# CMU-SAFARI/PyGim

Measured on AMD Instinct MI355X. Metric: SpMM GFLOP/s, Reddit-shaped CSR h=256 fp32, higher is better.
Workload: dtype f32

## Files before the change

### pygim_amd/autotune.py

```python
from __future__ import annotations

import math
from dataclasses import dataclass

RATE_PANEL = 17.0e12
RATE_GATHER_FAR = 4.8e12
RATE_GATHER_MALL = 7.0e12
RATE_STREAM = 5.0e12
XGMI_IN = 7 * 45e9
PANEL_BYTES = 4 << 20
LAUNCH = 6e-6
CUS = 256
LDS_ROWS_MAX = 8 * 228
LDS_NS_PER_COLUMN = 3.43
LDS_NS_PER_ENTRY = 0.26
LDS_NS_PER_ENTRY_HALF = 0.5
LDS_NS_PER_COLUMN_FLOOR = 4.4
LDS_COL_SPLIT = True
LDS_ROW_TAIL = 3
TAIL_S = 30e-6
LDS_MIN_LANES = 5
LDS_MIN_REUSE_NARROW = 0.75
LDS_HALF_SPLIT = True
LDS_MIN_REUSE = 0.75


@dataclass
class Choice:
    row_parts: int
    feat_parts: int
    seconds: float
    product_s: float
    collective_s: float
    panel: bool


def lds_rows_per_tile(nrows, nslices, rmax=LDS_ROWS_MAX, cus=CUS):
    tiles = -(-nrows // rmax)
    wgs = tiles * nslices
    rounds = -(-wgs // cus)
    if rounds > 8:
        return rmax
    if wgs % cus == 0:
        return -(-nrows // tiles)
    tiles2 = rounds * cus // nslices
    if tiles2 <= tiles:
        return rmax
    return min(rmax, max(16, -(-nrows // tiles2)))


def lds_product_seconds(nrows, ncols, nnz, h, es):
    if es != 4 or h < LDS_MIN_LANES or nrows == 0 or nnz == 0:
        return None
    nsl = -(-h // 64)
    pack_s = ncols * h * es * 2 / RATE_STREAM
    cols_x = ncols
    ns_entry = LDS_NS_PER_ENTRY
    if LDS_HALF_SPLIT and h * es <= 128 and ncols >= 4 * 128:
        cols_x = -(-ncols // 2)
        ns_entry = LDS_NS_PER_ENTRY_HALF
    min_reuse = LDS_MIN_REUSE if h * es > 128 else max(LDS_MIN_REUSE, LDS_MIN_REUSE_NARROW * (1.6 if cols_x != ncols else 1.0))
    tall = -(-int(nrows) // LDS_ROWS_MAX)
    split = min(8, CUS // (tall * nsl)) if tall * nsl * 2 <= CUS else 1
    tail_rows = 0
    if LDS_COL_SPLIT and nnz >= (1 << 20):
        for s2 in range(8, split, -1):
            tall_s = CUS // (nsl * s2)
            if not tall_s:
                continue
            covered = tall_s * LDS_ROWS_MAX
            if covered >= nrows:
                break
            if (nrows - covered) * 100 <= nrows * LDS_ROW_TAIL and tall_s * nsl * s2 * 10 >= CUS * 9:
                split, tall, tail_rows = s2, tall_s, nrows - covered
                break
    if LDS_COL_SPLIT and nnz >= (1 << 20) and split > 1:
        if nnz / (tall * cols_x) < min_reuse:
            return None
        tall2 = CUS // (nsl * split)
        if not tail_rows and tall < tall2 <= 2 * tall:
            tall = tall2
        per_wg = max(cols_x / split * LDS_NS_PER_COLUMN + nnz / tall / split * ns_entry, cols_x / split * LDS_NS_PER_COLUMN_FLOOR) * 1e-9
        reduce_s = (split + 1) * nrows * h * es / RATE_STREAM
        return per_wg + reduce_s + pack_s + 2 * LAUNCH + (TAIL_S if tail_rows else 0.0)
    rpt = lds_rows_per_tile(int(nrows), nsl)
    tiles = -(-int(nrows) // rpt)
    if nnz / (tiles * cols_x) < min_reuse:
        return None
    per_wg = max(cols_x * LDS_NS_PER_COLUMN + nnz / tiles * ns_entry, cols_x * LDS_NS_PER_COLUMN_FLOOR) * 1e-9
    rounds = -(-tiles * nsl // CUS)
    return rounds * per_wg + pack_s + LAUNCH


def product_seconds(nrows, ncols, nnz, h, es):
    if nrows == 0 or nnz == 0 or h == 0:
        return 0.0, False
    t_lds = lds_product_seconds(nrows, ncols, nnz, h, es)
    if t_lds is not None:
        return t_lds, True
    row_bytes = h * es
    line_bytes = max(row_bytes, 128) if row_bytes < 128 else row_bytes
    gather = nnz * line_bytes
    npanels = max(1, math.ceil(ncols * 128 / PANEL_BYTES))
    panel = row_bytes >= 64 and (npanels == 1 or nnz / (nrows * npanels) >= 8)
    if panel:
        nsl = math.ceil(row_bytes / 128)
        t = gather / RATE_PANEL + npanels * (2 * nrows * row_bytes) / RATE_STREAM / 8 + nsl * 4 * nnz / RATE_STREAM / 8
        t += npanels * LAUNCH + ncols * row_bytes * 2 / RATE_STREAM
    else:
        x_bytes = ncols * row_bytes
        rate = RATE_GATHER_MALL if x_bytes <= 300e6 else RATE_GATHER_FAR
        t = gather / rate + LAUNCH
    return t, panel


def price(nrows, ncols, nnz, h, es, row_parts, feat_parts):
    hp = math.ceil(h / feat_parts)
    t, panel = product_seconds(math.ceil(nrows / row_parts), ncols, nnz / row_parts, hp, es)
    gpus = row_parts * feat_parts
    coll = 0.0 if gpus == 1 else (nrows * h * es) * (1 - 1 / gpus) / XGMI_IN
    return Choice(row_parts, feat_parts, t + coll, t, coll, panel)


def choose(nrows, ncols, nnz, h, elem_bytes, n_gpus):
    table = []
    for r in range(1, n_gpus + 1):
        if n_gpus % r:
            continue
        f = n_gpus // r
        if f > h:
            continue
        table.append(price(nrows, ncols, nnz, h, elem_bytes, r, f))
    best = min(table, key=lambda c: c.seconds)
    return best, table


def autotune(nrows, ncols, nnz, hidden_size, elem_bytes=4, n_gpus=8):
    best, _ = choose(nrows, ncols, nnz, hidden_size, elem_bytes, n_gpus)
    return [best.row_parts, best.feat_parts, "nnz", "nnz", None]


def autotune_dataset(datadir, dataset, hidden_size, split_set, blnc_set=(0, 2), elem_bytes=4):
    from . import datasets, synth

    assert len(split_set) > 0 and len(blnc_set) > 0
    got = datasets.load_adjacency(datadir, dataset)
    if got is not None:
        nrows, nnz = int(got[2]), int(len(got[1]))
    else:
        nrows, nnz, _ = synth.DATASETS[dataset]
    best = None
    for sp, ds in split_set:
        if sp < 1 or ds < 1 or ds > hidden_size:
            continue
        c = price(nrows, nrows, nnz, hidden_size, elem_bytes, sp, ds)
        if best is None or c.seconds < best.seconds:
            best = c
    if best is None:
        return [None, None, None, None, None]
    return [best.row_parts, best.feat_parts, "nnz", "nnz", None]
```

### pygim_amd/csrc/kernels.hpp

```cpp
#pragma once
#include <hip/hip_runtime.h>
#include <stdint.h>
#include <type_traits>

namespace pygim {

template <typename T> struct AccOf { using type = T; };
template <> struct AccOf<int8_t> { using type = uint32_t; };
template <> struct AccOf<int16_t> { using type = uint32_t; };
template <> struct AccOf<int32_t> { using type = uint32_t; };
template <> struct AccOf<int64_t> { using type = uint64_t; };

template <typename T> __device__ __forceinline__ typename AccOf<T>::type to_acc(T v) {
    using A = typename AccOf<T>::type;
    if constexpr (std::is_floating_point<T>::value) return v;
    else if constexpr (sizeof(T) == 8) return (A)v;
    else return (A)(int32_t)v;
}
template <typename T> __device__ __forceinline__ T from_acc(typename AccOf<T>::type a) {
    if constexpr (std::is_floating_point<T>::value) return a;
    else return (T)a;
}

__device__ __forceinline__ uint32_t rfl(uint32_t v) { return __builtin_amdgcn_readfirstlane(v); }
// ... 721 lines not shown
    const uint32_t f = (uint32_t)(i % w);
    using A = typename AccOf<T>::type;
    A acc = (A)part[r * ldp + f];
    for (uint32_t c = 1; c < splits; c++) acc = (A)(acc + (A)part[((uint64_t)c * nrows + r) * ldp + f]);
    float y = (float)(T)acc * (1.0f * quant_scale(*absmax_bits, log2_range));
    if (post_mul) {
        y = post_mul[f] * y + post_add[f];
        if (post_relu) y = fmaxf(y, 0.0f);
    }
    out[r * ldo + f] = y;
}

template <typename T, bool DEQ>
__global__ void k_lds_reduce_v4(const T *__restrict__ part, uint32_t splits, uint64_t nrows, uint32_t w, uint64_t ldp, void *__restrict__ C, int64_t ldc, int accumulate,
                                const uint32_t *__restrict__ absmax_bits, int log2_range, const float *__restrict__ post_mul, const float *__restrict__ post_add, int post_relu) {
    static_assert(sizeof(T) == 4, "4-byte element types");
    using A = typename AccOf<T>::type;
    const uint32_t w4 = w >> 2;
    const uint64_t i = (uint64_t)blockIdx.x * blockDim.x + threadIdx.x;
    if (i >= nrows * w4) return;
    const uint64_t r = i / w4;
    const uint32_t f = (uint32_t)(i % w4) * 4;
    T v[4];
    load_vec<T, 4>(part + r * ldp + f, v);
    A acc[4];
#pragma unroll
    for (int k = 0; k < 4; k++) acc[k] = to_acc<T>(v[k]);
    for (uint32_t c = 1; c < splits; c++) {
        load_vec<T, 4>(part + ((uint64_t)c * nrows + r) * ldp + f, v);
#pragma unroll
        for (int k = 0; k < 4; k++) acc[k] = (A)(acc[k] + to_acc<T>(v[k]));
    }
    if constexpr (DEQ) {
        const float scale = 1.0f * quant_scale(*absmax_bits, log2_range);
        float y[4];
#pragma unroll
        for (int k = 0; k < 4; k++) {
            y[k] = (float)from_acc<T>(acc[k]) * scale;
            if (post_mul) {
                y[k] = post_mul[f + k] * y[k] + post_add[f + k];
                if (post_relu) y[k] = fmaxf(y[k], 0.0f);
            }
        }
        store_vec<float, 4>((float *)C + r * ldc + f, y);
    } else {
        T *c = (T *)C + r * ldc + f;
        if (accumulate) {
            load_vec<T, 4>(c, v);
#pragma unroll
            for (int k = 0; k < 4; k++) acc[k] = (A)(to_acc<T>(v[k]) + acc[k]);
        }
#pragma unroll
        for (int k = 0; k < 4; k++) v[k] = from_acc<T>(acc[k]);
        store_vec<T, 4>(c, v);
    }
}

template <int MODE>
__global__ void k_lds_reduce16(const int16_t *__restrict__ part, uint32_t splits, uint64_t nrows, uint32_t w, uint64_t ldp, void *__restrict__ C, int64_t ldc, int accumulate,
                               const uint32_t *__restrict__ absmax_bits, int log2_range, const float *__restrict__ post_mul, const float *__restrict__ post_add, int post_relu) {
    const uint64_t i = (uint64_t)blockIdx.x * blockDim.x + threadIdx.x;
    if (i >= nrows * w) return;
    const uint64_t r = i / w;
    const uint32_t f = (uint32_t)(i % w);
    uint32_t acc = (uint32_t)(int32_t)part[r * ldp + f];
    for (uint32_t c = 1; c < splits; c++) acc += (uint32_t)(int32_t)part[((uint64_t)c * nrows + r) * ldp + f];
    if constexpr (MODE == 0) {
        int8_t *c8 = (int8_t *)C + (int64_t)r * ldc + f;
        if (accumulate) acc += (uint32_t)(int32_t)*c8;
        *c8 = (int8_t)acc;
    } else {
        float y = (float)(MODE == 1 ? (int32_t)(int8_t)acc : (int32_t)(int16_t)acc) * (1.0f * quant_scale(*absmax_bits, log2_range));
        if (post_mul) {
            y = post_mul[f] * y + post_add[f];
            if (post_relu) y = fmaxf(y, 0.0f);
        }
        ((float *)C)[(int64_t)r * ldc + f] = y;
    }
}

constexpr uint32_t LDS_TAIL_SEG = 256;
template <typename T>
__global__ __launch_bounds__(512) void k_lds_tail_seg(const uint32_t *__restrict__ segs, uint32_t nseg, const uint32_t *__restrict__ colind, const char *__restrict__ xs,
                                                      uint64_t slice_stride, typename AccOf<T>::type *__restrict__ parked) {
    static_assert(sizeof(T) == 4, "4-byte element types");
    using A = typename AccOf<T>::type;
    __shared__ A partial[8][64];
    const uint32_t seg = blockIdx.x, slice = blockIdx.y;
    const uint32_t wave = threadIdx.x >> 6, lane = threadIdx.x & 63;
    const uint32_t e0 = segs[nseg + seg], e1 = segs[2 * nseg + seg];
    const char *xsl = xs + (uint64_t)slice * slice_stride + lane * 4;
    static_assert(LDS_TAIL_SEG == 256, "32 entries per wave");
    uint32_t cols[32];
#pragma unroll
    for (int k = 0; k < 32; k++) {
        const uint32_t e = e0 + wave + 8u * k;
        cols[k] = e < e1 ? colind[e] : 0xFFFFFFFFu;
    }
    T x[32];
#pragma unroll
    for (int k = 0; k < 32; k++) x[k] = cols[k] != 0xFFFFFFFFu ? *(const T *)(xsl + (uint64_t)cols[k] * 256) : (T)0;
    A acc = 0;
#pragma unroll
    for (int k = 0; k < 32; k++) acc = (A)(acc + to_acc<T>(x[k]));
    partial[wave][lane] = acc;
    __syncthreads();
    if (wave != 0) return;
    A sum = partial[0][lane];
#pragma unroll
    for (int v = 1; v < 8; v++) sum = (A)(sum + partial[v][lane]);
    parked[((uint64_t)seg * gridDim.y + slice) * 64 + lane] = sum;
}
template <typename T, bool DEQ>
__global__ __launch_bounds__(64) void k_lds_tail_fin(const uint32_t *__restrict__ rowseg, uint32_t row0, const typename AccOf<T>::type *__restrict__ parked, uint32_t w_lanes,
                                                     void *__restrict__ C, int64_t ldc_bytes, int accumulate, const uint32_t *__restrict__ absmax_bits, int log2_range,
                                                     const float *__restrict__ post_mul, const float *__restrict__ post_add, int post_relu) {
    using A = typename AccOf<T>::type;
    const uint32_t t = blockIdx.x, slice = blockIdx.y, lane = threadIdx.x;
    const uint32_t f = slice * 64 + lane;
    if (f >= w_lanes) return;
    A sum = 0;
    for (uint32_t s = rowseg[t]; s < rowseg[t + 1]; s++) sum = (A)(sum + parked[((uint64_t)s * gridDim.y + slice) * 64 + lane]);
    const uint64_t row = (uint64_t)row0 + t;
    if constexpr (DEQ) {
        float y = (float)from_acc<T>(sum) * (1.0f * quant_scale(*absmax_bits, log2_range));
        if (post_mul) {
            y = post_mul[f] * y + post_add[f];
            if (post_relu) y = fmaxf(y, 0.0f);
        }
        *(float *)((char *)C + (int64_t)row * ldc_bytes + (size_t)f * 4) = y;
    } else {
        T *c = (T *)((char *)C + (int64_t)row * ldc_bytes + (size_t)f * 4);
        if (accumulate) sum = (A)(to_acc<T>(*c) + sum);
        *c = from_acc<T>(sum);
    }
}

__global__ void k_copy16(const u32x4_t *__restrict__ src, u32x4_t *__restrict__ dst, uint64_t n) {
    const uint64_t i = (uint64_t)blockIdx.x * blockDim.x + threadIdx.x;
    if (i < n) dst[i] = src[i];
}

template <typename T>
__global__ void k_narrow_vals(const T *__restrict__ vals, uint64_t n, typename NarrowOf<T>::type *__restrict__ narrow, int *flag) {
    using NT = typename NarrowOf<T>::type;
    const uint64_t i = (uint64_t)blockIdx.x * blockDim.x + threadIdx.x;
    if (i >= n) return;
    const T v = vals[i];
    const NT q = (NT)v;
    bool same;
    if constexpr (std::is_same<T, double>::value) same = __double_as_longlong((double)q) == __double_as_longlong(v);
    else same = (T)q == v;
    narrow[i] = q;
    if (!same) atomicOr(flag, 1);
}

template <typename T>
__global__ void k_widen_vals(const T *__restrict__ vals, uint64_t n, uint32_t *__restrict__ wide) {
    const uint64_t i = (uint64_t)blockIdx.x * blockDim.x + threadIdx.x;
    if (i < n) wide[i] = (uint32_t)(int32_t)vals[i];
}

template <typename T, int VEC, int LOG_LPR, int AMODE, int HAS_VALS, bool DEQ = false>
__global__ __launch_bounds__(256) void k_csr_panel(const uint32_t *__restrict__ item_row,
                                                   const uint32_t *__restrict__ item_begin,
                                                   const uint32_t *__restrict__ item_len, uint32_t nitems,
                                                   const uint32_t *__restrict__ coop_row,
                                                   const uint32_t *__restrict__ coop_begin,
                                                   const uint32_t *__restrict__ coop_len, uint32_t ncoop,
                                                   uint32_t coop_grid, const uint32_t *__restrict__ colind,
                                                   const T *__restrict__ vals, const T *__restrict__ X,
                                                   int64_t ldx, int64_t slice_stride, T *__restrict__ C,
                                                   int64_t ldc, uint32_t w, uint32_t nslices, int accumulate,
                                                   uint32_t col_base, float *__restrict__ Cf, int64_t ldcf,
                                                   const uint32_t *__restrict__ absmax_bits, int log2_range,
                                                   const float *__restrict__ post_mul, const float *__restrict__ post_add,
                                                   int post_relu) {
    static_assert(LOG_LPR == 3, "lane groups of 8 (one 128-byte line per gathered row slice)");
    if (blockIdx.x < coop_grid)
        panel_sweep<T, VEC, AMODE, HAS_VALS, true, DEQ>(blockIdx.x, coop_row, coop_begin, coop_len, ncoop, colind, vals, X,
                                                        ldx, slice_stride, C, ldc, w, nslices, accumulate, col_base, Cf, ldcf,
                                                        absmax_bits, log2_range, post_mul, post_add, post_relu);
    else
        panel_sweep<T, VEC, AMODE, HAS_VALS, false, DEQ>(blockIdx.x - coop_grid, item_row, item_begin, item_len, nitems,
// ... 675 lines not shown
```

### pygim_amd/csrc/lds_codegen.hpp

```cpp
#pragma once
#include <stdint.h>

#include <algorithm>
#include <stdexcept>
#include <vector>

#include "lds_plan.hpp"

#if defined(__HIPCC__)
#define PYGIM_HD __host__ __device__
#else
#define PYGIM_HD
#endif

namespace pygim {

struct CgParams {
    uint32_t NW = 8, KA = 228, KC = 128, NBUF = 5, RB = 256, RPB = 256, G = 10, NS = 2, XW = 1;
    uint32_t wide = 0, valued = 0;
    uint32_t mulw = 0;
    uint32_t int_inline = 0;
    uint32_t i64_full = 0;
    uint32_t opcode_add = 0x02000000u, addw = 1;
    uint32_t pieces = 4, chunk_bytes = 32768;
    uint32_t nrows = 0, ncols = 0, nchunks = 0, ntiles = 0, nstreams = 0;
    uint32_t S = 1, row_tiles = 0;
    uint32_t col_bits = 1;
    uint32_t half_H = 0;
    uint32_t x0 = 6, acc0 = 28, vbase0 = 1, vbase1 = 2, vbase2 = 3, vl16 = 4, vtouch = 4, vjunk = 5;
    uint32_t s_xs = 80, s_ldsw = 82, s_cb = 84, s_ret = 86, s_pa = 92;
    PYGIM_HD uint32_t vbase(uint32_t blk) const { return blk == 0 ? vbase0 : blk == 1 ? vbase1 : vbase2; }
};

constexpr uint32_t CG_TOUCH_EVERY_DW = 256;

inline CgParams cg_params(const LdsGeometry &geo, uint32_t opcode_add, bool valued, uint32_t nrows, uint32_t ncols, uint32_t gsize = 0, uint32_t nsets = 0,
                          bool int_inline = false, bool i64_full = false, uint32_t half_H = 0) {
    if (geo.NBUF >= 3 && !geo.boundary) throw std::runtime_error("lds codegen: the mid-slot hand-off takes the host encoder");
    CgParams P;
    const bool wide = geo.row_bytes == 512;
    if (geo.row_bytes != 256 && geo.row_bytes != 512) throw std::runtime_error("lds codegen: rows of 256 or 512 bytes");
    if (wide != (opcode_add == LDS_CODE_ADD_F64 || opcode_add == LDS_CODE_ADD_U64)) throw std::runtime_error("lds codegen: 512-byte rows are the 8-byte element types'");
    const LdsCodeRegs R = lds_code_regs(geo.NW, gsize, nsets, wide);
    P.NW = geo.NW; P.KA = geo.KA; P.KC = geo.KC; P.NBUF = geo.NBUF; P.RB = geo.row_bytes; P.RPB = 65536 / geo.row_bytes;
    P.G = R.gsize; P.NS = R.nsets; P.XW = wide ? 2 : 1; P.wide = wide; P.valued = valued;
    if (R.x0 + R.nx() > R.acc0 || R.acc0 + P.KA * P.XW > 256 || P.G > 12 || (P.NS - 1) * P.G > 15 || P.NS > 8)
        throw std::runtime_error("lds codegen: the geometry does not fit the register map");
    if (P.KA > 255) throw std::runtime_error("lds codegen: more than 255 accumulators per wave");
    P.opcode_add = opcode_add;
    P.i64_full = (valued && opcode_add == LDS_CODE_ADD_U64 && i64_full) ? 1 : 0;
    P.int_inline = (valued && (opcode_add == 0x68000000u || opcode_add == LDS_CODE_ADD_U64 || opcode_add == LDS_CODE_PK_ADD_U16) && int_inline && !P.i64_full) ? 1 : 0;
    P.mulw = !valued ? 0 : opcode_add == LDS_CODE_ADD_F64 ? 6 : opcode_add == LDS_CODE_ADD_U64 ? (P.i64_full ? 12 : P.int_inline ? 6 : 8) : ((opcode_add == 0x68000000u || opcode_add == LDS_CODE_PK_ADD_U16) && !int_inline) ? 4 : 2;
    P.addw = (opcode_add == LDS_CODE_PK_ADD_U16 || opcode_add == LDS_CODE_ADD_F64 || opcode_add == LDS_CODE_ADD_U64) ? 2 : 1;
    if (valued && opcode_add == LDS_CODE_ADD_U64) P.addw = 0;
    P.pieces = (geo.KC * geo.row_bytes / 1024) / geo.NW;
    if (P.pieces * geo.NW * 1024 != geo.KC * geo.row_bytes) throw std::runtime_error("lds codegen: a chunk is not a whole number of pieces per wave");
    P.chunk_bytes = geo.KC * geo.row_bytes;
    if ((geo.KC * geo.NBUF + P.RPB - 1) / P.RPB > 3) throw std::runtime_error("lds codegen: the ring is larger than three 64 KiB blocks");
    if (geo.NBUF > 12) throw std::runtime_error("lds codegen: more than 12 ring buffers");
    if ((geo.half_split != 0) != (half_H != 0)) throw std::runtime_error("lds codegen: a half-split plan names its H (and only such a plan does)");
    if (half_H && (valued || wide || half_H % geo.KC || ncols != half_H)) throw std::runtime_error("lds codegen: half-split plans are unit-weight plans of 4-byte types over H = whole chunks of virtual columns");
    P.half_H = half_H;
    P.nrows = nrows; P.ncols = ncols;
    P.nchunks = (ncols + geo.KC - 1) / geo.KC;
    const uint32_t R_rows = geo.rows_per_tile ? std::min(geo.rows_per_tile, geo.NW * geo.KA) : geo.NW * geo.KA;
    P.S = std::max(1u, geo.col_splits);
    P.row_tiles = (nrows + R_rows - 1) / R_rows;
    P.ntiles = P.row_tiles * P.S;
    P.nstreams = P.ntiles * geo.NW;
    if ((uint64_t)nrows * P.S >= (1ull << 32)) throw std::runtime_error("lds codegen: rows x column ranges beyond 32 bits");
    P.col_bits = 1;
    while (P.col_bits < 32 && (1ull << P.col_bits) < (uint64_t)ncols) P.col_bits++;
    uint32_t sb = 1;
    while ((1ull << sb) < (uint64_t)P.nstreams) sb++;
    if (sb + P.col_bits + 8 > 64) throw std::runtime_error("lds codegen: key wider than 64 bits");
    P.x0 = R.x0; P.acc0 = R.acc0; P.vbase0 = R.vbase[0]; P.vbase1 = R.vbase[1]; P.vbase2 = R.vbase[2];
    P.vl16 = R.vl16; P.vtouch = R.vtouch; P.vjunk = R.vjunk;
    P.s_xs = R.s_xs; P.s_ldsw = R.s_ldsw; P.s_cb = R.s_cb; P.s_ret = R.s_ret; P.s_pa = R.s_pa;
    return P;
}
inline uint32_t cg_key_bits(const CgParams &P) {
    uint32_t sb = 1;
    while ((1ull << sb) < (uint64_t)P.nstreams) sb++;
    return sb + P.col_bits + 8;
}

struct CgRows {
    std::vector<uint32_t> rowinfo;
    std::vector<uint32_t> rowmap_rt;
    std::vector<uint32_t> tnnz;
    std::vector<uint32_t> tile_pos;
    std::vector<uint32_t> rowmap;
    std::vector<uint32_t> tile_row0, tile_nnz;
};
inline void cg_deal_rows_a(const uint32_t *rowptr, const LdsGeometry &geo, const CgParams &P, CgRows &out, const uint32_t *rorder = nullptr) {
    auto rid = [&](uint32_t pos) { return rorder ? rorder[pos] : pos; };
    auto rlen = [&](uint32_t pos) { const uint32_t r = rid(pos); return rowptr[r + 1] - rowptr[r]; };
    const uint32_t NW = geo.NW, KA = geo.KA, KAS = geo.ka_stride(), RS = NW * KAS;
    const uint32_t R = geo.rows_per_tile ? std::min(geo.rows_per_tile, NW * KA) : NW * KA;
    const uint32_t nrows = P.nrows, nrt = P.row_tiles;
    out.rowinfo.assign(nrows, 0);
    out.rowmap_rt.assign((size_t)nrt * RS, 0xFFFFFFFFu);
    out.tnnz.assign((size_t)nrt * P.S, 0);
    lds_parallel_for(nrt, 0, [&](uint32_t rt) {
        std::vector<uint32_t> order;
        const uint32_t r0 = rt * R, r1 = std::min(nrows, r0 + R), nr = r1 - r0;
        if (P.S == 1) {
            if (!rorder) out.tnnz[rt] = rowptr[r1] - rowptr[r0];
            else
                for (uint32_t q = r0; q < r1; q++) out.tnnz[rt] += rlen(q);
        }
        order.resize(nr);
        for (uint32_t i = 0; i < nr; i++) order[i] = i;
        std::stable_sort(order.begin(), order.end(), [&](uint32_t a, uint32_t b) { return rlen(r0 + a) > rlen(r0 + b); });
        for (uint32_t i = 0; i < nr; i++) {
            const uint32_t round = i / NW, p = i % NW;
            const uint32_t w = (round & 1) ? NW - 1 - p : p;
            out.rowinfo[rid(r0 + order[i])] = ((rt * NW + w) << 8) | round;
            out.rowmap_rt[((size_t)rt * NW + w) * KAS + round] = rid(r0 + order[i]);
        }
    });
}
inline void cg_deal_rows_b(const LdsGeometry &geo, const CgParams &P, CgRows &out) {
    const uint32_t NW = geo.NW, KAS = geo.ka_stride(), RS = NW * KAS;
    const uint32_t R = geo.rows_per_tile ? std::min(geo.rows_per_tile, NW * geo.KA) : NW * geo.KA;
    const uint32_t ntiles = P.ntiles;
    std::vector<uint32_t> ord(ntiles);
    for (uint32_t t = 0; t < ntiles; t++) ord[t] = t;
    if (!geo.keep_tile_order) std::stable_sort(ord.begin(), ord.end(), [&](uint32_t a, uint32_t b) { return out.tnnz[a] > out.tnnz[b]; });
    out.tile_pos.assign(ntiles, 0);
    for (uint32_t i = 0; i < ntiles; i++) out.tile_pos[ord[i]] = i;
    out.rowmap.assign((size_t)ntiles * RS, 0xFFFFFFFFu);
    out.tile_row0.assign(ntiles, 0);
    out.tile_nnz.assign(ntiles, 0);
    for (uint32_t t = 0; t < ntiles; t++) {
        const uint32_t rt = t / P.S, cs = t % P.S, ti = out.tile_pos[t];
        out.tile_row0[ti] = rt * R;
        out.tile_nnz[ti] = out.tnnz[t];
        for (uint32_t q = 0; q < RS; q++) {
            const uint32_t r = out.rowmap_rt[(size_t)rt * RS + q];
            if (r != 0xFFFFFFFFu) out.rowmap[(size_t)ti * RS + q] = r + cs * P.nrows;
        }
    }
}

// ... 124 lines not shown
    }
    const uint32_t ch = T.chunks[T.choff[s / P.NW] + j];
    const uint64_t target = ((uint64_t)s << (P.col_bits + 8)) | ((uint64_t)ch * P.KC << 8);
    uint64_t lo = 0, hi = T.nnz;
    while (lo < hi) {
        const uint64_t mid = (lo + hi) >> 1;
        if (T.keys[mid] < target) lo = mid + 1;
        else hi = mid;
    }
    T.slot_firstcol[sj] = lo < T.nnz ? T.colx[lo] : T.ncols_total;
}
PYGIM_HD inline void cg_slot_ngroups(const CgParams &P, const CgTables &T, uint32_t sj) {
    const uint32_t m = T.slot_firstcol[sj + 1] - T.slot_firstcol[sj];
    T.slot_ng[sj] = (m + P.G - 1) / P.G;
}
PYGIM_HD inline unsigned long long cg_slot_groups(const CgParams &P, const CgTables &T, uint32_t sj) {
    const uint32_t c0 = T.slot_firstcol[sj], c1 = T.slot_firstcol[sj + 1];
    uint32_t g = T.slot_firstgroup[sj];
    unsigned long long pairs = 0;
    for (uint32_t c = c0; c < c1; c += P.G, g++) {
        const uint32_t ce = c + P.G < c1 ? c + P.G : c1;
        uint32_t nlds = 0;
        for (uint32_t u = 0; c + u < ce; u++) {
            T.col_g[c + u] = (g << 4) | u;
            if (P.wide) { nlds++; continue; }
            if ((u & 1) == 0) {
                const bool paired = c + u + 1 < c1 && (T.col_lrow[c + u + 1] / P.RPB) == (T.col_lrow[c + u] / P.RPB);
                if (paired) {
                    nlds++;
                    pairs += (unsigned long long)(T.col_first[c + u + 2] - T.col_first[c + u]);
                } else {
                    nlds += (c + u + 1 < ce) ? 2 : 1;
                }
            }
        }
        T.g_first[g] = T.col_first[c];
        T.g_nent[g] = T.col_first[ce] - T.col_first[c];
        if (P.half_H) {
            uint32_t n0 = 0;
            for (uint32_t i = T.col_first[c]; i < T.col_first[ce]; i++) n0 += T.vals[i] == 0u;
            T.g_n0[g] = n0;
        }
        T.g_firstcol[g] = c;
        T.g_nlds[g] = (uint8_t)nlds;
        T.g_ncols[g] = (uint8_t)(ce - c);
    }
    return pairs;
}

struct CgEmit {
    uint32_t *out;
    uint64_t n;
    uint32_t since_touch;
    uint64_t vm_touch;
    PYGIM_HD void put(uint32_t a) {
        if (out) out[n] = a;
        n++;
    }
    PYGIM_HD void op(uint32_t a) { put(a); since_touch++; }
    PYGIM_HD void op(uint32_t a, uint32_t b) { put(a); put(b); since_touch += 2; }
    PYGIM_HD void skip(uint32_t dw) { n += dw; since_touch += dw; }
};

PYGIM_HD inline void cg_stream_pass(const CgParams &P, const CgTables &T, uint32_t s, bool write) {
    const uint32_t ti = s / P.NW;
    const uint32_t nch = T.nch[ti];
    const uint32_t *chunk_ids = T.chunks + T.choff[ti];
    const uint32_t sj0 = cg_sbase(P, T, s);
    CgEmit e;
    const uint64_t base_dw = write ? T.start[s] / 4 : 0;
    e.out = write ? T.code + base_dw : nullptr;
    e.n = 0;
    e.since_touch = 0;
    e.vm_touch = 0;
    auto s_add_lit = [&](uint32_t sdst, uint32_t ssrc, uint32_t lit) { e.op(0x80000000u | (sdst << 16) | (0xFFu << 8) | ssrc, lit); };
    auto s_addc0 = [&](uint32_t sdst, uint32_t ssrc) { e.op(0x82000000u | (sdst << 16) | (0x80u << 8) | ssrc); };
    auto touch = [&]() {
        s_add_lit(P.s_cb, P.s_cb, (e.since_touch + 5) * 4);
        s_addc0(P.s_cb + 1, P.s_cb + 1);
        e.op(0xDC508000u, (P.vjunk << 24) | (P.s_cb << 16) | P.vtouch);
        e.since_touch = 0;
        e.vm_touch++;
    };
    auto dma = [&](uint32_t cid, uint32_t buf) {
        s_add_lit(P.s_pa, P.s_xs, cid * P.chunk_bytes);
        s_addc0(P.s_pa + 1, P.s_xs + 1);
        for (uint32_t i = 0; i < P.pieces; i++) {
            if (i % 4 == 0) {
                if (i) {
                    s_add_lit(P.s_pa, P.s_pa, 0x1000);
                    s_addc0(P.s_pa + 1, P.s_pa + 1);
                }
                s_add_lit(124 , P.s_ldsw, buf * P.chunk_bytes + (i / 4) * 0x1000);
                e.op(0xBF800000u);
            }
            e.op(0xDDF48000u | ((i % 4) * 1024), (P.s_pa << 16) | P.vl16);
        }
    };
    uint64_t dma_issued = 0;
    uint64_t landed_mark[16];
    for (int q = 0; q < 16; q++) landed_mark[q] = 0;
    auto vm_now = [&]() { return dma_issued + e.vm_touch; };
    auto dma_chunk = [&](uint32_t j) {
        dma(chunk_ids[j], j % P.NBUF);
        dma_issued += P.pieces;
        landed_mark[j & 15] = vm_now();
    };
    auto wait_landed = [&](uint32_t j) {
        const uint64_t younger = vm_now() - landed_mark[j & 15];
        const uint32_t nn = (uint32_t)(younger < 63 ? younger : 63);
        e.op(0xBF8C0F70u | (nn & 15) | (((nn >> 4) & 3) << 14));
    };
    auto wait_lgkm = [&](uint32_t n) { e.op(0xBF8CC07Fu | ((n < 15u ? n : 15u) << 8)); };
    uint32_t pend_g[10], pend_nlds[10], npend = 0;
    uint32_t gcount = 0;
    auto consume_oldest = [&]() {
        uint32_t younger = 0;
        for (uint32_t q = 1; q < npend; q++) younger += pend_nlds[q];
        wait_lgkm(younger);
        const uint32_t g = pend_g[0];
        if (write) T.g_apos[g] = (uint32_t)(base_dw + e.n);
        e.skip(T.g_nent[g] * (P.mulw + P.addw));
        if (P.half_H) e.skip((T.g_n0[g] > 0 ? 1u : 0u) + (T.g_n0[g] < T.g_nent[g] ? 1u : 0u) + 1u);
        for (uint32_t q = 1; q < npend; q++) {
            pend_g[q - 1] = pend_g[q];
            pend_nlds[q - 1] = pend_nlds[q];
        }
        npend--;
    };
    if (nch) {
        for (uint32_t j = 0; j + 1 < P.NBUF && j < nch; j++) dma_chunk(j);
        wait_landed(0);
        e.op(0xBF8A0000u);
    }
    for (uint32_t j = 0; j < nch; j++) {
        bool dma_due = j + P.NBUF - 1 < nch;
        const uint32_t g0 = T.slot_firstgroup[sj0 + j], g1 = T.slot_firstgroup[sj0 + j + 1];
        for (uint32_t g = g0; g < g1; g++) {
            const uint32_t nlds = T.g_nlds[g];
            if (write) {
                T.g_rpos[g] = (uint32_t)(base_dw + e.n);
                T.g_xset[g] = (uint8_t)(gcount % P.NS);
            }
            e.skip(2 * nlds);
            pend_g[npend] = g;
            pend_nlds[npend] = nlds;
            npend++;
            gcount++;
            if (dma_due) {
                dma_chunk(j + P.NBUF - 1);
                dma_due = false;
            }
            if (npend >= P.NS) consume_oldest();
            if (e.since_touch >= CG_TOUCH_EVERY_DW) touch();
        }
        if (dma_due) dma_chunk(j + P.NBUF - 1);
        while (npend > 1) consume_oldest();
        wait_lgkm(0);
        if (j + 1 < nch) wait_landed(j + 1);
        e.op(0xBF8A0000u);
    }
    while (npend) consume_oldest();
    e.op(0xBF8C0F70u);
    e.op(0xBE801D00u | P.s_ret);
    while (e.n % 64) e.put(0xBF800000u);
    if (!write) T.stream_dw[s] = (uint32_t)e.n;
}

PYGIM_HD inline void cg_emit_reads(const CgParams &P, const CgTables &T, uint32_t g) {
    if (P.half_H) {
        uint32_t *a = T.code + T.g_apos[g];
        const uint32_t n0 = T.g_n0[g], n1 = T.g_nent[g] - n0;
        uint32_t at = 0;
        if (n0) { a[at] = 0xBEFE0100u | 76u; at += 1 + n0 * P.addw; }
        if (n1) { a[at] = 0xBEFE0100u | 78u; at += 1 + n1 * P.addw; }
        a[at] = 0xBEFE01C1u;
    }
    const uint32_t c0 = T.g_firstcol[g], nc = T.g_ncols[g];
    const uint32_t xb = P.x0 + P.G * P.XW * T.g_xset[g];
    uint32_t *w = T.code + T.g_rpos[g];
    for (uint32_t u = 0; u < nc;) {
        const uint32_t r0 = T.col_lrow[c0 + u], blk = r0 / P.RPB;
        if (P.wide) {
            *w++ = 0xD8EC0000u | ((r0 % P.RPB) * P.RB);
            *w++ = ((xb + u * 2) << 24) | P.vbase(blk);
            u++;
        } else if ((u & 1) == 0 && u + 1 < nc && (T.col_lrow[c0 + u + 1] / P.RPB) == blk) {
            const uint32_t r1 = T.col_lrow[c0 + u + 1];
// ... 196 lines not shown
```

### pygim_amd/csrc/lds_plan.hpp

```cpp
#pragma once
#include <stdint.h>
#if defined(__HIPCC__)
#define PYGIM_LDS_HD_INLINE __host__ __device__ inline
#else
#define PYGIM_LDS_HD_INLINE inline
#endif

#include <algorithm>
#include <atomic>
#include <cstdio>
#include <cstdlib>
#include <memory>
#include <stdexcept>
#include <thread>
#include <vector>

namespace pygim {

struct LdsTile {
    uint32_t nch;
    uint32_t chunk_off;
    uint32_t nb_off;
    uint32_t row0;
    uint32_t nnz;
    uint32_t chunk0;
    uint32_t pad[2];
    uint32_t tokstart[16];
};

constexpr uint32_t LDS_TOK_SLACK = 4096 + 64;

constexpr uint32_t LDS_HDR_SHIFT = 18, LDS_HDR_MAX = 0x3FFFu;

struct LdsGeometry {
    uint32_t NW = 8;
    uint32_t KA = 208;
    uint32_t KC = 320;
    uint32_t BATCH = 16;
    uint32_t rows_per_tile = 0;
    uint32_t keep_tile_order = 0;
    uint32_t col_splits = 1;
    uint32_t ka_stride() const { return (KA + 7) & ~7u; }
    uint32_t row_bytes = 256;
    uint32_t boundary = 0;
    uint32_t half_split = 0;
    uint32_t NBUF = 2;
};

struct LdsPlanHost {
    LdsGeometry geo;
    uint32_t ntiles = 0, nchunks = 0;
    uint64_t ntokens = 0;
    uint64_t slots = 0;
    std::vector<uint32_t> tok;
    std::vector<uint32_t> wts;
    std::vector<uint32_t> nb, chunks, rowmap;
    std::vector<LdsTile> tiles;
    std::atomic<bool> header_overflow{false};
};

inline unsigned lds_default_threads() {
    static const unsigned cached = [] {
        unsigned hw = std::max(1u, std::thread::hardware_concurrency());
        long long quota = -1, period = 100000;
        if (FILE *f = fopen("/sys/fs/cgroup/cpu.max", "r")) {
            char q[32] = {0};
            if (fscanf(f, "%31s %lld", q, &period) == 2 && q[0] != 'm') quota = atoll(q);
            fclose(f);
        } else if (FILE *g = fopen("/sys/fs/cgroup/cpu/cpu.cfs_quota_us", "r")) {
            if (fscanf(g, "%lld", &quota) != 1) quota = -1;
            fclose(g);
            if (FILE *h = fopen("/sys/fs/cgroup/cpu/cpu.cfs_period_us", "r")) {
                if (fscanf(h, "%lld", &period) != 1) period = 100000;
                fclose(h);
            }
        }
        if (quota > 0 && period > 0) hw = (unsigned)std::min<long long>(hw, std::max<long long>(1, (quota + period - 1) / period));
        return hw;
    }();
    return cached;
}

template <typename F> inline void lds_parallel_for(uint32_t n, unsigned threads, F &&fn) {
    if (threads == 0) threads = lds_default_threads();
    threads = std::min<unsigned>(threads, std::max(1u, n));
    std::atomic<uint32_t> next(0);
    std::atomic<bool> failed(false);
    auto body = [&]() {
        try {
            for (;;) {
                const uint32_t i = next.fetch_add(1);
                if (i >= n || failed.load(std::memory_order_relaxed)) return;
                fn(i);
            }
        } catch (...) {
            failed.store(true);
        }
    };
    std::vector<std::thread> pool;
    try {
        for (unsigned i = 1; i < threads; i++) pool.emplace_back(body);
    } catch (...) {
    }
    body();
    for (auto &th : pool) th.join();
    if (failed.load()) throw std::runtime_error("lds plan: a worker failed (out of memory?)");
}

inline void lds_plan_build(const uint32_t *rowptr, const uint32_t *col, uint32_t nrows, uint32_t ncols, const LdsGeometry &geo,
                           LdsPlanHost &out, unsigned threads = 0, const uint32_t *vals = nullptr, const uint32_t *rorder = nullptr) {
    auto rid = [&](uint32_t pos) { return rorder ? rorder[pos] : pos; };
    auto rlen = [&](uint32_t pos) { const uint32_t r = rid(pos); return rowptr[r + 1] - rowptr[r]; };
    const uint32_t NW = geo.NW, KA = geo.KA, KC = geo.KC, B = geo.BATCH;
    const uint32_t KAS = geo.ka_stride();
    const uint32_t RS = NW * KAS;
    const uint32_t R = geo.rows_per_tile ? std::min(geo.rows_per_tile, NW * KA) : NW * KA;
    const uint32_t S = std::max(1u, geo.col_splits);
    const uint32_t ntiles = ((nrows + R - 1) / R) * S;
    const uint32_t nchunks = (ncols + KC - 1) / KC;
    out.geo = geo;
    out.ntiles = ntiles;
    out.nchunks = nchunks;
    out.tiles.assign(ntiles, LdsTile());
    out.rowmap.assign((size_t)ntiles * RS, 0xFFFFFFFFu);

    struct TileTmp {
        std::vector<uint32_t> chunk_ids;
        std::vector<uint32_t> cnt;
        std::vector<uint8_t> wave_of;
        std::vector<uint16_t> k_of;
        uint64_t batches[16] = {0, 0, 0, 0, 0, 0, 0, 0, 0, 0, 0, 0, 0, 0, 0, 0};
    };
    std::vector<TileTmp> tmp(ntiles);
    auto run = [&](auto &&fn) { lds_parallel_for(ntiles, threads, fn); };
    run([&](uint32_t t) {
        TileTmp &tt = tmp[t];
        const uint32_t rt = t / S, cs = t % S;
        const uint32_t ch_lo = (uint32_t)((uint64_t)nchunks * cs / S), ch_hi = (uint32_t)((uint64_t)nchunks * (cs + 1) / S);
        const uint32_t r0 = rt * R, r1 = std::min(nrows, r0 + R), nr = r1 - r0;
        std::vector<uint32_t> order(nr);
        for (uint32_t i = 0; i < nr; i++) order[i] = i;
        std::stable_sort(order.begin(), order.end(), [&](uint32_t a, uint32_t b) {
            return rlen(r0 + a) > rlen(r0 + b);
        });
        tt.wave_of.resize(nr);
        tt.k_of.resize(nr);
        for (uint32_t i = 0; i < nr; i++) {
            const uint32_t round = i / NW, pos = i % NW;
            const uint32_t w = (round & 1) ? NW - 1 - pos : pos;
            tt.wave_of[order[i]] = (uint8_t)w;
            tt.k_of[order[i]] = (uint16_t)round;
            out.rowmap[((size_t)t * NW + w) * KAS + round] = rid(r0 + order[i]) + cs * nrows;
        }
        std::vector<uint32_t> cnt((size_t)nchunks * NW, 0);
        for (uint32_t i = 0; i < nr; i++) {
            const uint32_t w = tt.wave_of[i];
            for (uint32_t e = rowptr[rid(r0 + i)]; e < rowptr[rid(r0 + i) + 1]; e++) {
                const uint32_t ch = col[e] / KC;
                if (ch >= ch_lo && ch < ch_hi) cnt[(size_t)ch * NW + w]++;
            }
        }
        uint32_t nnz_range = 0;
        for (uint32_t c = 0; c < nchunks; c++) {
            uint32_t any = 0;
            for (uint32_t w = 0; w < NW; w++) any |= cnt[(size_t)c * NW + w];
            if (!any) continue;
            tt.chunk_ids.push_back(c);
            for (uint32_t w = 0; w < NW; w++) {
                const uint32_t n = cnt[(size_t)c * NW + w];
                nnz_range += n;
                tt.cnt.push_back(n);
                tt.batches[w] += std::max<uint32_t>(1, (n + B - 1) / B);
            }
        }
        out.tiles[t].nch = (uint32_t)tt.chunk_ids.size();
        out.tiles[t].chunk0 = tt.chunk_ids.empty() ? 0 : tt.chunk_ids[0];
        out.tiles[t].row0 = r0;
        out.tiles[t].nnz = nnz_range;
    });
    uint64_t tokb = 0, nbo = 0, cho = 0, slots = 0;
    for (uint32_t t = 0; t < ntiles; t++) {
        LdsTile &d = out.tiles[t];
        d.chunk_off = (uint32_t)cho;
        d.nb_off = (uint32_t)nbo;
        cho += d.nch + 2;
        nbo += (uint64_t)(d.nch + 2) * NW;
        slots += d.nch;
        for (uint32_t w = 0; w < NW; w++) {
            d.tokstart[w] = (uint32_t)tokb;
            tokb += tmp[t].batches[w];
        }
    }
    out.slots = slots;
    out.ntokens = tokb * B;
    out.tok.assign((size_t)out.ntokens + LDS_TOK_SLACK, KA);
    if (vals) out.wts.assign(out.tok.size(), 0u);
    else out.wts.clear();
    out.nb.assign((size_t)nbo + 256, 0);
    out.chunks.assign((size_t)cho + 128, 0);
    run([&](uint32_t t) {
        TileTmp &tt = tmp[t];
        const LdsTile &d = out.tiles[t];
        const uint32_t rt = t / S, cs = t % S;
        const uint32_t r0 = rt * R, r1 = std::min(nrows, r0 + R), nr = r1 - r0, nch = d.nch;
        for (uint32_t j = 0; j < nch + 2; j++) out.chunks[(size_t)d.chunk_off + j] = nch ? tt.chunk_ids[std::min(j, nch - 1)] : 0;
// ... 25 lines not shown
                }
            }
        for (uint32_t w = 0; w < NW; w++) {
            uint64_t at = (uint64_t)d.tokstart[w] * B;
            for (uint32_t j = 0; j < nch; j++) {
                const uint32_t nbj = batches_of(j, w), nbn = batches_of(j + 1, w), cidn = j + 1 < nch ? tt.chunk_ids[j + 1] : 0;
                if (nbj > LDS_HDR_MAX || nbn > LDS_HDR_MAX || cidn > LDS_HDR_MAX) out.header_overflow = true;
                out.tok[at] |= nbj << LDS_HDR_SHIFT;
                out.tok[at + 1] |= nbn << LDS_HDR_SHIFT;
                out.tok[at + 2] |= cidn << LDS_HDR_SHIFT;
                at += (uint64_t)nbj * B;
            }
        }
        (void)nr;
    });
    std::vector<uint32_t> ord(ntiles);
    for (uint32_t t = 0; t < ntiles; t++) ord[t] = t;
    if (!geo.keep_tile_order) std::stable_sort(ord.begin(), ord.end(), [&](uint32_t a, uint32_t b) { return out.tiles[a].nnz > out.tiles[b].nnz; });
    std::vector<LdsTile> tiles2(ntiles);
    std::vector<uint32_t> rowmap2(out.rowmap.size());
    for (uint32_t i = 0; i < ntiles; i++) {
        tiles2[i] = out.tiles[ord[i]];
        std::copy(out.rowmap.begin() + (size_t)ord[i] * RS, out.rowmap.begin() + (size_t)(ord[i] + 1) * RS, rowmap2.begin() + (size_t)i * RS);
    }
    out.tiles.swap(tiles2);
    out.rowmap.swap(rowmap2);
}

inline uint32_t lds_rows_per_tile(uint32_t nrows, uint32_t rmax, uint32_t nslices, uint32_t cus) {
    if (!nrows || !nslices || !cus) return rmax;
    const uint64_t tiles = (nrows + rmax - 1) / rmax, wgs = tiles * nslices;
    const uint64_t rounds = (wgs + cus - 1) / cus;
    if (rounds > 8) return rmax;
    if (wgs % cus == 0) return (uint32_t)((nrows + tiles - 1) / tiles);
    const uint64_t tiles2 = rounds * cus / nslices;
    if (tiles2 <= tiles) return rmax;
    return (uint32_t)std::min<uint64_t>(rmax, std::max<uint64_t>(16, (nrows + tiles2 - 1) / tiles2));
}

inline double lds_plan_uniform_reuse(uint64_t nnz, uint32_t nrows, uint32_t ncols, const LdsGeometry &geo) {
    const uint64_t R = geo.rows_per_tile ? geo.rows_per_tile : (uint64_t)geo.NW * geo.KA;
    const uint64_t ntiles = (nrows + R - 1) / R;
    if (!ntiles || !ncols) return 0;
    return (double)nnz / ((double)ntiles * (double)ncols);
}


struct LdsCodeRegs {
    uint32_t vbase[3] = {0, 0, 0};
    uint32_t vl16 = 0;
    uint32_t vtouch = 0;
    uint32_t vjunk = 0;
    uint32_t x0 = 0;
    uint32_t gsize = 0, nsets = 0;
    uint32_t acc0 = 0;
    uint32_t s_xs = 80;
    uint32_t s_ldsw = 82;
    uint32_t s_cb = 84;
    uint32_t s_ret = 86;
    uint32_t s_pa = 92;
    uint32_t wide = 0;
    constexpr uint32_t nx() const { return gsize * nsets * (wide ? 2 : 1); }
};
constexpr LdsCodeRegs lds_code_regs(uint32_t NW, uint32_t gsize = 0, uint32_t nsets = 0, bool wide = false) {
    LdsCodeRegs r;
    r.wide = wide ? 1 : 0;
    if (NW == 16) {
        r.vbase[0] = 4; r.vbase[1] = 5; r.vbase[2] = 10;
        r.vl16 = 6; r.vtouch = 11; r.vjunk = 9; r.x0 = 12; r.acc0 = 28;
        r.gsize = gsize ? gsize : 8;
        r.nsets = nsets ? nsets : 2;
    } else {
        r.vbase[0] = 1; r.vbase[1] = 2; r.vbase[2] = 3;
        r.vl16 = 4; r.vtouch = 4; r.vjunk = 5; r.x0 = 6; r.acc0 = 28;
        r.gsize = gsize ? gsize : (wide ? 5 : 10);
        r.nsets = nsets ? nsets : 2;
    }
    if (!wide && (r.gsize & 1)) r.gsize--;
    if (r.gsize < 2) r.gsize = 2;
    if (r.nsets < 2) r.nsets = 2;
    while (r.x0 + r.nx() > r.acc0 && r.gsize > 2) r.gsize -= wide ? 1 : 2;
    return r;
}
constexpr uint32_t LDS_CODE_AUTO_WAVES = 8, LDS_CODE8_AUTO_NBUF = 5;
constexpr uint32_t LDS_CODE8_KA64 = 114;
constexpr uint32_t LDS_CODE8_KA = 228;

struct LdsWords {
    std::unique_ptr<uint32_t[]> p;
    size_t n = 0;
    void alloc(size_t words) { p.reset(new uint32_t[words]); n = words; }
    uint32_t *data() { return p.get(); }
    const uint32_t *data() const { return p.get(); }
    size_t size() const { return n; }
    uint32_t &operator[](size_t i) { return p[i]; }
    const uint32_t &operator[](size_t i) const { return p[i]; }
};

struct LdsCodeHost {
    LdsWords code;
    std::vector<uint64_t> start;
    uint64_t entries = 0;
    uint64_t pairs = 0;
    uint64_t shared = 0;
    LdsCodeRegs regs;
};

constexpr uint32_t LDS_CODE_PK_ADD_U16 = 0xFFFFFFFFu;
constexpr uint32_t LDS_CODE_ADD_F64 = 0xFFFFFFFEu, LDS_CODE_ADD_U64 = 0xFFFFFFFDu;
constexpr uint32_t LDS_CODE_S_VAL = 94;
inline bool lds_int_values_inline(const uint32_t *vals, uint64_t n) {
    for (uint64_t i = 0; i < n; i++) {
        const int32_t v = (int32_t)vals[i];
        if (v < -16 || v > 64) return false;
    }
    return true;
}
PYGIM_LDS_HD_INLINE uint32_t lds_inline_int(int32_t v) { return v >= 0 ? 128u + (uint32_t)v : 192u + (uint32_t)(-v); }
inline void lds_code_from_plan(const LdsPlanHost &plan, uint32_t opcode_add, LdsCodeHost &out, unsigned threads = 0, uint32_t gsize = 0,
                               uint32_t nsets = 0, uint32_t experiment = 0, const uint64_t *vals64 = nullptr) {
    const LdsGeometry &geo = plan.geo;
    const uint32_t NW = geo.NW, KA = geo.KA, B = geo.BATCH, KC = geo.KC;
    const uint32_t RB = geo.row_bytes;
    const bool wide = RB == 512;
    if (RB != 256 && RB != 512) throw std::runtime_error("lds code: rows of 256 or 512 bytes");
    if (wide != (opcode_add == LDS_CODE_ADD_F64 || opcode_add == LDS_CODE_ADD_U64)) throw std::runtime_error("lds code: 512-byte rows are the 8-byte element types'");
    if (!plan.wts.empty() && (opcode_add == LDS_CODE_ADD_F64 || opcode_add == LDS_CODE_ADD_U64) && !vals64)
        throw std::runtime_error("lds code: valued entries of this element type");
    const LdsCodeRegs R = lds_code_regs(NW, gsize, nsets, wide);
    out.regs = R;
    const uint32_t G = R.gsize, NS = R.nsets;
    if (R.x0 + R.nx() > R.acc0 || R.acc0 + KA * (wide ? 2 : 1) > 256 || G > 12 || (NS - 1) * G > 15)
        throw std::runtime_error("lds code: the geometry does not fit the register map");
    const uint32_t pieces = (KC * RB / 1024) / NW;
    if (pieces * NW * 1024 != KC * RB) throw std::runtime_error("lds code: a chunk is not a whole number of pieces per wave");
    const uint32_t chunk_bytes = KC * RB;
    const uint32_t RPB = 65536 / RB;
    if ((KC * geo.NBUF + RPB - 1) / RPB > 3) throw std::runtime_error("lds code: the ring is larger than three 64 KiB blocks");
    const uint32_t ntiles = plan.ntiles;
    constexpr uint32_t TOUCH_EVERY_DW = 256;

    struct Emit {
        uint32_t *out = nullptr;
        size_t n = 0;
        uint32_t since_touch = 0;
        uint64_t vm_touch = 0;
        void put(uint32_t a) {
            if (out) out[n] = a;
            n++;
        }
        void op(uint32_t a) { put(a); since_touch++; }
        void op(uint32_t a, uint32_t b) { put(a); put(b); since_touch += 2; }
    };
    struct Grp {
        uint32_t nx = 0, nlds = 0, xb = 0;
        std::vector<uint32_t> k, xr, v;
    };
    const LdsCodeRegs Rr = R;
    bool int_inline = (opcode_add == 0x68000000u || opcode_add == LDS_CODE_PK_ADD_U16) && !plan.wts.empty() && lds_int_values_inline(plan.wts.data(), plan.wts.size());
    bool i64_full = false;
    if (opcode_add == LDS_CODE_ADD_U64 && !plan.wts.empty()) {
        int_inline = true;
        for (uint64_t i = 0; i < plan.ntokens; i++) {
            if ((plan.tok[i] & 0xFF) >= KA) continue;
            const int64_t v = (int64_t)vals64[plan.wts[i]];
            if (v != (int64_t)(int32_t)v) i64_full = true;
            if (v < -16 || v > 64) int_inline = false;
        }
        if (i64_full) int_inline = false;
    }
    auto emit_stream = [&](uint32_t ti, uint32_t wv, Emit &e, uint64_t &n_entries, uint64_t &n_pairs, uint64_t &n_shared) {
        const LdsTile &t = plan.tiles[ti];
        auto s_add_lit = [&](uint32_t sdst, uint32_t ssrc, uint32_t lit) { e.op(0x80000000u | (sdst << 16) | (0xFFu << 8) | ssrc, lit); };
        auto s_addc0 = [&](uint32_t sdst, uint32_t ssrc) { e.op(0x82000000u | (sdst << 16) | (0x80u << 8) | ssrc); };
        auto touch = [&]() {
            s_add_lit(Rr.s_cb, Rr.s_cb, (e.since_touch + 5) * 4);
            s_addc0(Rr.s_cb + 1, Rr.s_cb + 1);
            e.op(0xDC508000u, (Rr.vjunk << 24) | (Rr.s_cb << 16) | Rr.vtouch);
            e.since_touch = 0;
            e.vm_touch++;
        };
        auto dma = [&](uint32_t cid, uint32_t buf) {
            s_add_lit(Rr.s_pa, Rr.s_xs, cid * chunk_bytes);
            s_addc0(Rr.s_pa + 1, Rr.s_xs + 1);
            for (uint32_t i = 0; i < pieces; i++) {
                if (i % 4 == 0) {
                    if (i) {
                        s_add_lit(Rr.s_pa, Rr.s_pa, 0x1000);
                        s_addc0(Rr.s_pa + 1, Rr.s_pa + 1);
                    }
                    s_add_lit(124 , Rr.s_ldsw, buf * chunk_bytes + (i / 4) * 0x1000);
                    e.op(0xBF800000u);
                }
                if (!(experiment & 2)) e.op(0xDDF48000u | ((i % 4) * 1024), (Rr.s_pa << 16) | Rr.vl16);
            }
        };
        uint64_t at = (uint64_t)t.tokstart[wv] * B;
        const uint32_t NBUF = geo.NBUF;
        const bool mid = NBUF >= 3 && !geo.boundary;
        uint64_t dma_issued = 0;
        auto vm_now = [&]() { return dma_issued + e.vm_touch; };
        std::vector<uint64_t> landed_mark(t.nch + NBUF + 1, 0);
        auto dma_chunk = [&](uint32_t j) {
            dma(plan.chunks[t.chunk_off + j], j % NBUF);
            dma_issued += (experiment & 2) ? 0 : pieces;
            landed_mark[j] = vm_now();
        };
        const bool spread = (experiment & 4) && pieces <= 4 && !mid;
        uint32_t dma_left = 0, dma_j = 0;
        auto dma_begin = [&](uint32_t j) {
            const uint32_t cid = plan.chunks[t.chunk_off + j], buf = j % NBUF;
            s_add_lit(Rr.s_pa, Rr.s_xs, cid * chunk_bytes);
            s_addc0(Rr.s_pa + 1, Rr.s_xs + 1);
            s_add_lit(124 , Rr.s_ldsw, buf * chunk_bytes);
            e.op(0xBF800000u);
            dma_left = pieces;
            dma_j = j;
        };
        auto dma_piece = [&]() {
            const uint32_t i = pieces - dma_left;
            e.op(0xDDF48000u | (i * 1024), (Rr.s_pa << 16) | Rr.vl16);
            dma_issued++;
            if (!--dma_left) landed_mark[dma_j] = vm_now();
        };
        auto wait_landed = [&](uint32_t j) {
            const uint64_t younger = vm_now() - landed_mark[j];
            const uint32_t nn = (uint32_t)std::min<uint64_t>(younger, 63);
            e.op(0xBF8C0F70u | (nn & 15) | (((nn >> 4) & 3) << 14));
        };
        auto wait_lgkm = [&](uint32_t n) { e.op(0xBF8CC07Fu | (std::min(n, 15u) << 8)); };
        const bool halves = geo.half_split != 0;
        const bool valued = !plan.wts.empty() && !halves;
        std::vector<Grp> ring(NS + 1);
        std::vector<uint32_t> pend;
        uint32_t gcount = 0;
        uint32_t lds_this_slot = 0;
        bool older_reads = false;
        auto consume_oldest = [&]() {
            uint32_t younger = 0;
            for (size_t q = 1; q < pend.size(); q++) younger += ring[pend[q]].nlds;
            wait_lgkm(younger);
            if (younger <= lds_this_slot) older_reads = false;
            const Grp &g = ring[pend.front()];
            if (valued && opcode_add == LDS_CODE_ADD_U64) {
                for (size_t q = 0; q < g.k.size(); q++) {
                    const uint64_t v64 = vals64[g.v[q]];
                    const int32_t v = (int32_t)(uint32_t)v64;
                    const uint32_t xl = g.xr[q], xh = g.xr[q] + 1, al = Rr.acc0 + g.k[q] * 2, ah = al + 1;
                    const uint32_t src = int_inline ? lds_inline_int(v) : LDS_CODE_S_VAL;
                    if (!int_inline) e.op(0xBE8000FFu | (LDS_CODE_S_VAL << 16), (uint32_t)v);
                    if (i64_full) e.op(0xBE8000FFu | ((LDS_CODE_S_VAL + 1) << 16), (uint32_t)(v64 >> 32));
                    e.op(0xD2850000u | xh, src | ((256 + xh) << 9));
                    if (!i64_full) e.op(v < 0 ? (0x6A000000u | (xh << 17) | (xl << 9) | (256 + xh)) : 0xBF800000u);
                    e.op(0x68000000u | (ah << 17) | (ah << 9) | (256 + xh));
                    if (i64_full) {
                        e.op(0xD2850000u | xh, (LDS_CODE_S_VAL + 1) | ((256 + xl) << 9));
                        e.op(0x68000000u | (ah << 17) | (ah << 9) | (256 + xh));
                    }
                    e.op(0xD1E86A00u | al, src | ((256 + xl) << 9) | ((256 + al) << 18));
                }
            } else if (valued && opcode_add == LDS_CODE_ADD_F64) {
                for (size_t q = 0; q < g.k.size(); q++) {
                    const uint64_t v = vals64[g.v[q]];
                    e.op(0xBE8000FFu | (LDS_CODE_S_VAL << 16), (uint32_t)v);
                    e.op(0xBE8000FFu | ((LDS_CODE_S_VAL + 1) << 16), (uint32_t)(v >> 32));
                    e.op(0xD2810000u | g.xr[q], LDS_CODE_S_VAL | ((256 + g.xr[q]) << 9));
                }
            } else if (valued && opcode_add == LDS_CODE_PK_ADD_U16) {
                for (size_t q = 0; q < g.k.size(); q++) {
                    if (!int_inline) e.op(0xBE8000FFu | (LDS_CODE_S_VAL << 16), g.v[q]);
                    e.op(0xD3814000u | g.xr[q], 0x10000000u | ((256 + g.xr[q]) << 9) | (int_inline ? lds_inline_int((int32_t)g.v[q]) : LDS_CODE_S_VAL));
                }
            } else if (valued && opcode_add == 0x68000000u) {
                for (size_t q = 0; q < g.k.size(); q++) {
                    if (int_inline) e.op(0xD2850000u | g.xr[q], lds_inline_int((int32_t)g.v[q]) | ((256 + g.xr[q]) << 9));
                    else {
                        e.op(0xBE8000FFu | (LDS_CODE_S_VAL << 16), g.v[q]);
                        e.op(0xD2850000u | g.xr[q], LDS_CODE_S_VAL | ((256 + g.xr[q]) << 9));
                    }
                }
            } else if (valued)
                for (size_t q = 0; q < g.k.size(); q++) e.op(0x0A0000FFu | (g.xr[q] << 17) | (g.xr[q] << 9), g.v[q]);
            for (uint32_t pass = 0; pass < (halves ? 2u : 1u); pass++) {
            if (halves) {
                bool any = false;
                for (size_t q = 0; q < g.k.size() && !any; q++) any = (g.v[q] & 1u) == pass;
                if (!any) continue;
                e.op(0xBEFE0100u | (pass ? 78u : 76u));
// ... 160 lines not shown
```

### pygim_amd/csrc/pygim_hip.hip

```cpp
#include "../../include/pygim_hip.h"
#include "kernels.hpp"
#ifdef PYGIM_LDS_ABLATE
#include "lds_kernel_gen_ablate.hpp"
#else
#include "lds_kernel_gen.hpp"
#include "lds_codegen_dev.hpp"
#include "lds_reorder_dev.hpp"
#include "lds_hybrid_dev.hpp"
#endif
#include "transpose_dev.hpp"
#include "sddmm_dev.hpp"
#include "spmm_values_dev.hpp"
#include "edge_softmax_dev.hpp"
#include <hsa/hsa.h>
#include <hsa/hsa_ext_amd.h>

static inline uint64_t lds_rows_pad(uint64_t ncols, uint32_t kc) {
    const uint64_t k = kc ? kc : 320;
    return ((ncols + k - 1) / k * k + 63) / 64 * 64;
}

#include <algorithm>
#include <atomic>
#include <chrono>
// ... 67 lines not shown
    }
    g_ctx.inited = false;
    g_ctx.generation++;
    return 0;
}

int64_t pygim_generation(void) { return g_ctx.generation; }

int pygim_device_info(char *name, int name_len, int *cu_count, int64_t *hbm_bytes) {
    int dev = 0;
    hipError_t e = hipGetDevice(&dev);
    if (e != hipSuccess) {
        (void)hipGetLastError();
        return fail(PYGIM_ERR_NO_DEVICE, "no HIP device visible");
    }
    hipDeviceProp_t prop;
    HIP_TRY(hipGetDeviceProperties(&prop, dev));
    if (name && name_len > 0) {
        std::snprintf(name, (size_t)name_len, "%s (%s)", prop.name, prop.gcnArchName);
    }
    if (cu_count) *cu_count = prop.multiProcessorCount;
    if (hbm_bytes) *hbm_bytes = (int64_t)prop.totalGlobalMem;
    return 0;
}

int64_t pygim_set_tunable(const char *name, int64_t value) {
    int64_t *slot = nullptr;
    std::string n = name ? name : "";
    if (n == "long_row_threshold") slot = &g_tune.long_row_threshold;
    else if (n == "long_segment") slot = &g_tune.long_segment;
    else if (n == "force_vec_bytes") slot = &g_tune.force_vec_bytes;
    else if (n == "csr_kernel") slot = &g_tune.csr_kernel;
    else if (n == "coo_chunk") slot = &g_tune.coo_chunk;
    else if (n == "coo_via_rowptr") slot = &g_tune.coo_via_rowptr;
    else if (n == "kernel_events") slot = &g_tune.kernel_events;
    else if (n == "host_windows") slot = &g_tune.host_windows;
    else if (n == "host_direct") slot = &g_tune.host_direct;
    else if (n == "panel_mode") slot = &g_tune.panel_mode;
    else if (n == "panel_bytes") slot = &g_tune.panel_bytes;
    else if (n == "panel_min_seg") slot = &g_tune.panel_min_seg;
    else if (n == "panel_pack") slot = &g_tune.panel_pack;
    else if (n == "panel_coop") slot = &g_tune.panel_coop;
    else if (n == "panel_block") slot = &g_tune.panel_block;
    else if (n == "slice_group_bytes") slot = &g_tune.slice_group_bytes;
    else if (n == "fuse_windows") slot = &g_tune.fuse_windows;
    else if (n == "panel_col16") slot = &g_tune.panel_col16;
    else if (n == "panel_locality") slot = &g_tune.panel_locality;
    else if (n == "split_unit_pattern") slot = &g_tune.split_unit_pattern;
    else if (n == "narrow_vals") slot = &g_tune.narrow_vals;
    else if (n == "merge_parts") slot = &g_tune.merge_parts;
    else if (n == "vec_kernel") slot = &g_tune.vec_kernel;
    else if (n == "vec_lds") slot = &g_tune.vec_lds;
    else if (n == "panel_lds_pad") slot = &g_tune.panel_lds_pad;
    else if (n == "vec_lds_min_seg") slot = &g_tune.vec_lds_min_seg;
    else if (n == "lds_mode") slot = &g_tune.lds_mode;
    else if (n == "lds_min_reuse_x100") slot = &g_tune.lds_min_reuse_x100;
    else if (n == "lds_min_width") slot = &g_tune.lds_min_width;
    else if (n == "lds_min_width8") slot = &g_tune.lds_min_width8;
    else if (n == "lds_min_reuse_narrow_x100") slot = &g_tune.lds_min_reuse_narrow_x100;
    else if (n == "lds_threads") slot = &g_tune.lds_threads;
    else if (n == "lds_waves") slot = &g_tune.lds_waves;
    else if (n == "lds_ablate") slot = &g_tune.lds_ablate;
    else if (n == "lds_round_tiles") slot = &g_tune.lds_round_tiles;
    else if (n == "lds_code") slot = &g_tune.lds_code;
    else if (n == "lds_code_nbuf") slot = &g_tune.lds_code_nbuf;
    else if (n == "lds_code_waves") slot = &g_tune.lds_code_waves;
    else if (n == "lds_fail") slot = &g_tune.lds_fail;
    else if (n == "lds_stamp") slot = &g_tune.lds_stamp;
    else if (n == "lds_code_exp") slot = &g_tune.lds_code_exp;
    else if (n == "lds_hybrid") slot = &g_tune.lds_hybrid;
    else if (n == "lds_hybrid_min") slot = &g_tune.lds_hybrid_min;
    else if (n == "lds_hybrid_contig") slot = &g_tune.lds_hybrid_contig;
    else if (n == "lds_code_boundary") slot = &g_tune.lds_code_boundary;
    else if (n == "lds_xcd_slices") slot = &g_tune.lds_xcd_slices;
    else if (n == "lds_codegen") slot = &g_tune.lds_codegen;
    else if (n == "lds_tile_order") slot = &g_tune.lds_tile_order;
    else if (n == "lds_lp_rounds") slot = &g_tune.lds_lp_rounds;
    else if (n == "lds_code_kc") slot = &g_tune.lds_code_kc;
    else if (n == "lds_code_gsize") slot = &g_tune.lds_code_gsize;
    else if (n == "lds_code_nsets") slot = &g_tune.lds_code_nsets;
    else if (n == "lds_col_split") slot = &g_tune.lds_col_split;
    else if (n == "lds_col_split_f32") slot = &g_tune.lds_col_split_f32;
    else if (n == "lds_fill_tiles") slot = &g_tune.lds_fill_tiles;
    else if (n == "lds_row_tail") slot = &g_tune.lds_row_tail;
    else if (n == "lds_split_order") slot = &g_tune.lds_split_order;
    else if (n == "lds_half_split") slot = &g_tune.lds_half_split;
    else if (n == "lds_direct_x") slot = &g_tune.lds_direct_x;
    else if (n == "lds_long_slots") slot = &g_tune.lds_long_slots;
    if (!slot) {
        fail(PYGIM_ERR_INVALID, "unknown tunable: " + n);
        return -1;
    }
    const int64_t old = *slot;
    if (slot == &g_tune.panel_lds_pad) value = std::min<int64_t>(std::max<int64_t>(value, 0), 64 << 10);
    *slot = value;
    return old;
}

}

static int group_create(int format, int dtype, int n_parts, const int32_t *const *idx0, const int32_t *const *colind,
                        const void *const *values, const int64_t *nrows, const int64_t *ncols, const int64_t *nnz,
                        const int64_t *n_dense, const int64_t *dense_cols, int64_t h_size, int64_t *out_handle, bool adopt) {
    bool adopted = false;
    auto drop_adopted = [&]() {
        if (!adopt || adopted) return;
        adopted = true;
        (void)hipFree(const_cast<int32_t *>(idx0[0]));
        (void)hipFree(const_cast<int32_t *>(colind[0]));
        if (values && values[0]) (void)hipFree(const_cast<void *>(values[0]));
    };
    if (int rc = need_init()) return drop_adopted(), rc;
    if (format != PYGIM_CSR && format != PYGIM_COO) return fail(PYGIM_ERR_INVALID, "format must be CSR(0) or COO(1)");
    const size_t es = dtype_size(dtype);
    if (es == 0) return fail(PYGIM_ERR_INVALID, "unknown dtype");
    if (n_parts <= 0 || !idx0 || !colind || !nrows || !ncols || !nnz || !n_dense || !dense_cols || !out_handle)
        return fail(PYGIM_ERR_INVALID, "null argument or n_parts <= 0");
    if (h_size <= 0) return fail(PYGIM_ERR_INVALID, "h_size must be positive");
    const double t0 = now_ms();
    Group *g = new Group;
    g->format = format;
    g->dtype = dtype;
    t_plan_dtype = dtype;
    g->h = h_size;
    g->total_rows = nrows[0];
    g->parts.resize(n_parts);
    hipStream_t st = nullptr;
    int rc = 0;
    auto bail = [&](int code) {
        (void)hipDeviceSynchronize();
        drop_adopted();
        free_group(g);
        return code;
    };
    if (hipMalloc((void **)&g->d_flags, 8 * sizeof(int)) != hipSuccess) return bail(fail(PYGIM_ERR_HIP, "hipMalloc flags"));
    if (hipMemsetAsync(g->d_flags, 0, 8 * sizeof(int), st) != hipSuccess) return bail(fail(PYGIM_ERR_HIP, "memset flags"));
    if (hipStreamCreateWithFlags(&g->side, hipStreamNonBlocking) != hipSuccess ||
        hipEventCreateWithFlags(&g->ev_fork, hipEventDisableTiming) != hipSuccess ||
        hipEventCreateWithFlags(&g->ev_join, hipEventDisableTiming) != hipSuccess)
        return bail(fail(PYGIM_ERR_HIP, "side stream / events"));
    size_t dpos = 0;
    for (int i = 0; i < n_parts; i++) {
        Part &p = g->parts[i];
        p.nrows = nrows[i];
        p.ncols = ncols[i];
        p.nnz = nnz[i];
        if (p.nrows != g->total_rows) return bail(fail(PYGIM_ERR_INVALID, "all sparse parts must have the same number of rows"));
        if (p.nrows < 0 || p.ncols < 0 || p.nnz < 0 || p.nnz > 0xFFFFFFFFll || p.nrows >= 0xFFFFFFFFll ||
            p.ncols > 0xFFFFFFFFll)
            return bail(fail(PYGIM_ERR_INVALID, "part sizes must fit 32-bit indices (the reference's uint32 matrices)"));
        if (n_dense[i] <= 0) return bail(fail(PYGIM_ERR_INVALID, "n_dense must be positive"));
        int64_t sum = 0;
        for (int64_t j = 0; j < n_dense[i]; j++) {
            if (dense_cols[dpos + j] < 0) return bail(fail(PYGIM_ERR_INVALID, "negative dense width"));
            p.dense_cols.push_back(dense_cols[dpos + j]);
            sum += dense_cols[dpos + j];
        }
        dpos += (size_t)n_dense[i];
        if (sum != h_size) return bail(fail(PYGIM_ERR_INVALID, "dense widths of a part must add up to h_size"));
        g->total_cols += p.ncols;
        if (!idx0[i] && (format == PYGIM_CSR || p.nnz > 0)) return bail(fail(PYGIM_ERR_INVALID, "null index array"));
        if (!colind[i] && p.nnz > 0) return bail(fail(PYGIM_ERR_INVALID, "null colind"));

        if ((rc = to_device<uint32_t>(colind[i], (size_t)p.nnz * 4, &p.colind, &p.own_colind, st))) return bail(rc);
        const void *v = values ? values[i] : nullptr;
        if (v) {
// ... 460 lines not shown
    out[1] = (int64_t)p.lds_slots;
    out[2] = (int64_t)p.lds_tokens;
    out[3] = p.nnz;
    return 0;
}

int pygim_group_lds_code(int64_t handle, int64_t out[4]) {
    Group *g = lookup(handle);
    if (!g) return fail(PYGIM_ERR_INVALID, "unknown group handle");
    const Part &p = (g->merged && g_tune.merge_parts && g->parts.size() > 1) ? *g->merged : g->parts[0];
    out[0] = p.lds_code ? (int64_t)p.lds_code_bytes : 0;
    out[1] = p.lds_code ? (int64_t)p.lds_code_pairs : 0;
    bool all_code = p.lds_is_code && g_tune.lds_code;
    if (!(g->merged && g_tune.merge_parts && g->parts.size() > 1))
        for (const Part &q : g->parts) all_code = all_code && q.lds_is_code;
    out[2] = all_code ? 1 : 0;
    out[3] = (p.lds_code && p.lds_codegen_device) ? 1 : 0;
    return 0;
}

int pygim_group_lds_tiles(int64_t handle, int64_t out[4]) {
    Group *g = lookup(handle);
    if (!g) return fail(PYGIM_ERR_INVALID, "unknown group handle");
    const Part &p = (g->merged && g_tune.merge_parts && g->parts.size() > 1) ? *g->merged : g->parts[0];
    out[0] = p.lds_tile_labels ? 1 : 0;
    out[1] = p.lds_tile_labels;
    out[2] = p.lds_tile_largest;
    out[3] = p.panel_locality_used ? p.sim_kind : 0;
    return 0;
}

int pygim_group_serial(int64_t handle, int64_t *out) {
    Group *g = lookup(handle);
    if (!g || !out) return fail(PYGIM_ERR_INVALID, "unknown group handle");
    *out = g->serial;
    return 0;
}

int pygim_group_lds_runs(int64_t handle, int64_t *out) {
    Group *g = lookup(handle);
    if (!g || !out) return fail(PYGIM_ERR_INVALID, "unknown group handle");
    *out = g->lds_runs;
    return 0;
}

int pygim_group_host_windows(int64_t handle, int64_t *windows, int64_t *direct) {
    Group *g = lookup(handle);
    if (!g || !windows) return fail(PYGIM_ERR_INVALID, "unknown group handle");
    *windows = g->host_windows_used;
    if (direct) *direct = g->host_direct_used;
    return 0;
}

int pygim_group_lds_geometry(int64_t handle, int64_t out[8]) {
    Group *g = lookup(handle);
    if (!g) return fail(PYGIM_ERR_INVALID, "unknown group handle");
    const Part &p = (g->merged && g_tune.merge_parts && g->parts.size() > 1) ? *g->merged : g->parts[0];
    for (int i = 0; i < 8; i++) out[i] = 0;
    if (!p.lds_tiles) return 0;
    out[0] = p.lds_nw;
    out[1] = p.lds_ka;
    out[2] = p.lds_kc;
    out[3] = p.lds_nbuf;
    out[4] = p.lds_is_code ? p.lds_code_gsize : 0;
    out[5] = p.lds_is_code ? p.lds_code_nsets : 0;
    out[6] = p.lds_is_code ? (int64_t)p.lds_code_shared : 0;
    out[7] = p.lds_col_splits;
    return 0;
}

int pygim_group_lds_note(int64_t handle, char *out, int64_t cap) {
    Group *g = lookup(handle);
    if (!g) return fail(PYGIM_ERR_INVALID, "unknown group handle");
    if (!out || cap <= 0) return fail(PYGIM_ERR_INVALID, "no buffer");
    std::string text;
    if ((g->merged && g_tune.merge_parts && g->parts.size() > 1) || g->parts.size() == 1) {
        text = ((g->merged && g_tune.merge_parts && g->parts.size() > 1) ? *g->merged : g->parts[0]).lds_note;
    } else {
        text = g->parts[0].lds_note;
        for (size_t i = 1; i < g->parts.size(); i++)
            if (g->parts[i].lds_note != g->parts[0].lds_note) text += "; part " + std::to_string(i) + ": " + g->parts[i].lds_note;
    }
    for (size_t i = 0; i < g->parts.size(); i++)
        if (!g->parts[i].hy_note.empty()) text += "; part " + std::to_string(i) + ": " + g->parts[i].hy_note;
    const size_t n = std::min<size_t>(text.size(), (size_t)cap - 1);
    std::memcpy(out, text.data(), n);
    out[n] = 0;
    return 0;
}

int pygim_group_info(int64_t handle, int64_t out[8]) {
    Group *g = lookup(handle);
    if (!g) return fail(PYGIM_ERR_INVALID, "unknown group handle");
    out[0] = g->total_rows;
    out[1] = g->total_cols;
    out[2] = g->h;
    out[3] = (int64_t)g->parts.size();
    int64_t nl = 0;
    for (auto &p : g->parts) nl += p.lp_base.n_long;
    out[4] = nl;
    out[5] = g->all_ones ? 1 : 0;
    out[6] = g->parts[0].d_items ? (int64_t)g->parts[0].npanels : 0;
    out[7] = (int64_t)g->parts[0].n_items;
    return 0;
}

int pygim_block_run_x(int64_t handle, int part, const void *X, int64_t ldx, void *C, int64_t ldc, int64_t width,
                      int accumulate, int x_unchanged, void *stream) {
    if (int rc = need_init()) return rc;
    Group *g = lookup(handle);
    if (!g) return fail(PYGIM_ERR_INVALID, "unknown group handle");
    if (part < 0 || part >= (int)g->parts.size()) return fail(PYGIM_ERR_INVALID, "part index out of range");
    if (!X || !C || width <= 0 || ldx < width || ldc < width) return fail(PYGIM_ERR_INVALID, "bad X/C/width/stride");
    if (!is_device_ptr(X) || !is_device_ptr(C)) return fail(PYGIM_ERR_INVALID, "pygim_block_run needs device pointers");
    g->x_unchanged = x_unchanged != 0;
    const int rc = launch_block_any(g, g->parts[part], X, ldx, C, ldc, width, accumulate != 0, (hipStream_t)stream);
    g->x_unchanged = false;
    return rc;
}

int pygim_block_run(int64_t handle, int part, const void *X, int64_t ldx, void *C, int64_t ldc, int64_t width,
                    int accumulate, void *stream) {
    return pygim_block_run_x(handle, part, X, ldx, C, ldc, width, accumulate, 0, stream);
}

int pygim_spmm_run_group_x(int64_t handle, const void *const *B_parts, void *out, int x_unchanged, void *stream) {
    if (int rc = need_init()) return rc;
    Group *g = lookup(handle);
    if (!g) return fail(PYGIM_ERR_INVALID, "unknown group handle");
    for (auto &p : g->parts)
        if (p.dense_cols != g->parts[0].dense_cols)
            return fail(PYGIM_ERR_INVALID, "spmm_run_group needs the same dense split for every sparse part");
    g->x_unchanged = x_unchanged != 0;
    const int rc = run_group_common(g, B_parts, nullptr, false, out, (hipStream_t)stream);
    g->x_unchanged = false;
    return rc;
}

int pygim_spmm_run_group(int64_t handle, const void *const *B_parts, void *out, void *stream) {
    return pygim_spmm_run_group_x(handle, B_parts, out, 0, stream);
}

int pygim_grande_run_group(int64_t handle, const void *const *B_windows, const int64_t *window_ld, void *out,
                           void *stream) {
    if (int rc = need_init()) return rc;
    Group *g = lookup(handle);
    if (!g) return fail(PYGIM_ERR_INVALID, "unknown group handle");
    if (!window_ld) return fail(PYGIM_ERR_INVALID, "window_ld is required");
    return run_group_common(g, B_windows, window_ld, true, out, (hipStream_t)stream);
}

int pygim_spmv_run_group(int64_t handle, const void *const *B_vectors, void *out, void *stream) {
    if (int rc = need_init()) return rc;
    Group *g = lookup(handle);
    if (!g) return fail(PYGIM_ERR_INVALID, "unknown group handle");
    hipStream_t st = (hipStream_t)stream;
    const size_t es = dtype_size(g->dtype);
    const size_t nvec = g->parts[0].dense_cols.size();
    for (auto &p : g->parts) {
        if (p.dense_cols.size() != nvec) return fail(PYGIM_ERR_INVALID, "spmv group: dense split differs between parts");
        for (auto wdt : p.dense_cols)
            if (wdt != 1) return fail(PYGIM_ERR_INVALID, "spmv group: every dense part must be one column wide");
    }
    if (!B_vectors || !out) return fail(PYGIM_ERR_INVALID, "null vectors or output");
    for (size_t j = 0; j < nvec; j++)
        if (!B_vectors[j]) return fail(PYGIM_ERR_INVALID, "null vector");
// ... 82 lines not shown
```

### pygim_amd/csrc/rt_launch.inc

```
int pick_vec_bytes(size_t es, const void *X, int64_t ldx, const void *C, int64_t ldc) {
    auto ok = [&](size_t vb) {
        return ((uintptr_t)X % vb == 0) && ((uintptr_t)C % vb == 0) && ((size_t)ldx * es % vb == 0) &&
               ((size_t)ldc * es % vb == 0);
    };
    size_t cap = g_tune.force_vec_bytes > 0 ? (size_t)g_tune.force_vec_bytes : 16;
    for (size_t vb : {(size_t)16, (size_t)8})
        if (vb <= cap && vb > es && ok(vb)) return (int)vb;
    return (int)es;
}

struct KernelTimer {
    Group *g;
    hipStream_t st;
    hipEvent_t a = nullptr, b = nullptr;
    KernelTimer(Group *g_, hipStream_t st_, bool on = true) : g(g_), st(st_) {
        if (on && (g_tune.kernel_events || g->kernel_events) && hipEventCreate(&a) == hipSuccess && hipEventCreate(&b) == hipSuccess)
            (void)hipEventRecord(a, st);
        else
            a = b = nullptr;
    }
    void stop() {
        if (!a) return;
        (void)hipEventRecord(b, st);
        g->ev_pending.emplace_back(a, b);
// ... 165 lines not shown
                       (AM == 3 ? (const uint32_t *)p.col16 : p.colind), vals, Xs0, ldg,                                  \
                       slice_stride, Cs0, ldc, ws, ns, (accumulate ? 1 : 0) | (p.panel_locality_used ? 2 : 0), q * p.panel_cols,   \
                       g->deq_out ? g->deq_out + (size_t)s0 * F : nullptr, g->deq_ld, g->deq_amax, g->deq_log2,                  \
                       g->post_mul ? g->post_mul + (size_t)s0 * F : nullptr, g->post_add ? g->post_add + (size_t)s0 * F : nullptr, \
                       g->post_relu)
#define PYGIM_LAUNCH_PANEL(AM, HV) PYGIM_LAUNCH_PANEL_D(AM, HV, false)
                int amode = !off32 ? 0 : ((size_t)ldg * sizeof(T) == 128 ? 2 : 1);
                if (amode == 2 && p.col16 && g_tune.panel_col16) amode = 3;
                if constexpr (DeqType<T>::ok) {
                    if (g->deq_out && amode >= 2 && !vals) {
                        if (amode == 3) PYGIM_LAUNCH_PANEL_D(3, 0, true);
                        else PYGIM_LAUNCH_PANEL_D(2, 0, true);
                        continue;
                    }
                }
                if (g->deq_out) return fail(PYGIM_ERR_INVALID, "internal: fused dequantisation on an unsupported sweep");
                if constexpr (sizeof(T) == 8) {
                    if (vals && p.vals_narrow && g_tune.narrow_vals) {
                        const T *vals = (const T *)p.vals_narrow;
                        if (amode == 3) PYGIM_LAUNCH_PANEL(3, 2);
                        else if (amode == 2) PYGIM_LAUNCH_PANEL(2, 2);
                        else if (amode == 1) PYGIM_LAUNCH_PANEL(1, 2);
                        else PYGIM_LAUNCH_PANEL(0, 2);
                        continue;
                    }
                }
                if (amode == 3 && vals) PYGIM_LAUNCH_PANEL(3, 1);
                else if (amode == 3) PYGIM_LAUNCH_PANEL(3, 0);
                else if (amode == 2 && vals) PYGIM_LAUNCH_PANEL(2, 1);
                else if (amode == 2) PYGIM_LAUNCH_PANEL(2, 0);
                else if (amode == 1 && vals) PYGIM_LAUNCH_PANEL(1, 1);
                else if (amode == 1) PYGIM_LAUNCH_PANEL(1, 0);
                else if (vals) PYGIM_LAUNCH_PANEL(0, 1);
                else PYGIM_LAUNCH_PANEL(0, 0);
#undef PYGIM_LAUNCH_PANEL
#undef PYGIM_LAUNCH_PANEL_D
            }
            }
            kt.stop();
            return join();
        }
    }
    bool wide = lanes_needed > 32;
    if (g_tune.csr_kernel == 1) wide = true;
    if (g_tune.csr_kernel == 2 && lanes_needed <= 32) wide = false;
    if (nrows > 0) {
        KernelTimer kt(g, st, !p.is_extra || p.timed);
        if (wide) {
            dim3 grid((nrows + 3) / 4, (lanes_needed + 63) / 64);
            hipLaunchKernelGGL((k_csr_wide<T, VEC>), grid, dim3(256), 0, st, p.rowptr, p.colind, vals, X, ldx, C,
                               ldc, nrows, w, lp.thresh, accumulate ? 1 : 0);
        } else {
            int log_lpr = 0;
            while ((1u << log_lpr) < lanes_needed) log_lpr++;
            const uint32_t rows_per_wave = 64u >> log_lpr;
            const uint32_t waves = (nrows + rows_per_wave - 1) / rows_per_wave;
            hipLaunchKernelGGL((k_csr_sub<T, VEC>), dim3((waves + 3) / 4), dim3(256), 0, st, p.rowptr, p.colind,
                               vals, X, ldx, C, ldc, nrows, w, lp.thresh, accumulate ? 1 : 0, log_lpr);
        }
        kt.stop();
    }
    return join();
}

template <typename T>
int launch_lds(Group *g, Part &p, const T *X, int64_t ldx, T *C, int64_t ldc, uint32_t w, bool accumulate, hipStream_t st,
               const void *lds_xs = nullptr, const uint32_t *deq_amax = nullptr, int deq_log2 = 0) {
    constexpr bool WIDE8 = sizeof(T) == 1;
    constexpr bool EL8 = sizeof(T) == 8;
    constexpr uint32_t ROWB = EL8 ? 512 : 256;
    constexpr uint32_t EPS = WIDE8 ? 128 : ROWB / sizeof(T);
    constexpr int PVEC = WIDE8 ? 8 : 16 / (int)sizeof(T);
    const bool split16 = p.lds_col_splits > 1 && (WIDE8 || (sizeof(T) == 2 && deq_amax != nullptr));
    const uint32_t w_lanes = split16 ? (uint32_t)(((size_t)w * 2 + 3) / 4)
                                     : (WIDE8 || EL8 || (sizeof(T) == 2 && deq_amax)) ? w : (uint32_t)(((size_t)w * sizeof(T) + 3) / 4);
    const bool HS = p.lds_half != 0;
    if (HS && (sizeof(T) != 4 || w > 32 || lds_xs || deq_amax)) return fail(PYGIM_ERR_INVALID, "internal: a half-split LDS plan serves plain 4-byte products of at most 32 lanes");
    const uint32_t nslices = HS ? 1u : (w + EPS - 1) / EPS;
    const uint64_t rows_pad = HS ? (uint64_t)p.lds_half : lds_rows_pad((uint64_t)p.ncols, p.lds_kc);
    const size_t need = (size_t)rows_pad * nslices * ROWB;
    KernelTimer kt(g, st, !p.is_extra || p.timed);
    XsPin pin;
    void *xs_use = const_cast<void *>(lds_xs);
    if (!xs_use && g_tune.lds_direct_x && nslices == 1 && !HS && !WIDE8 && !p.lds_col_order && (size_t)ldx * sizeof(T) == ROWB && (size_t)w * sizeof(T) == ROWB &&
        ((uintptr_t)X & 255) == 0) {
        void *base = nullptr;
        size_t size = 0;
        if (hipMemGetAddressRange((hipDeviceptr_t *)&base, &size, (hipDeviceptr_t)X) == hipSuccess && base && (const char *)X + (size_t)rows_pad * ROWB <= (const char *)base + size)
            xs_use = const_cast<void *>((const void *)X);
        else
            (void)hipGetLastError();
    }
    if (!xs_use) {
        std::lock_guard<std::mutex> lk(g_ctx.mu);
        if (g->x_unchanged) {
            int dev = 0;
            (void)hipGetDevice(&dev);
            Context::XsBuf *hit = nullptr;
            for (auto &kv : g_ctx.xs_bufs) {
                Context::XsBuf &b = kv.second;
                if (kv.first.first == dev && b.ptr && b.src == (const void *)X && b.ld == ldx && b.rows == p.ncols && b.w == (int64_t)w &&
                    b.es == sizeof(T) && b.kind == (HS ? 5 : WIDE8 ? 3 : 1) && b.rows_pad == rows_pad && b.order == (const void *)p.lds_col_order && b.bytes >= need &&
                    (!hit || b.stamp > hit->stamp))
                    hit = &b;
            }
            if (hit) {
                hit->stamp = ++g_ctx.xs_clock;
                hit->in_use++;
                xs_use = hit->ptr;
                pin.hold(xs_use);
            }
        }
        if (!xs_use) {
            Context::XsBuf *b = nullptr;
            if (int rc = xs_buffer_locked(st, std::max<size_t>(need, 256), &b)) return rc;
            xs_use = b->ptr;
            pin.hold(xs_use);
            b->src = X;
            b->ld = ldx;
            b->rows = p.ncols;
            b->w = (int64_t)w;
            b->es = sizeof(T);
            b->kind = HS ? 5 : WIDE8 ? 3 : 1;
            b->rows_pad = rows_pad;
            b->order = p.lds_col_order;
            const uint64_t threads = (uint64_t)p.ncols * nslices * 16;
            if (HS) {
                if constexpr (sizeof(T) == 4) {
                    const uint64_t th = rows_pad * 16;
                    hipLaunchKernelGGL((k_slice_pack_hs<T>), dim3((unsigned)((th + 255) / 256)), dim3(256), 0, st, X, ldx, (uint32_t)p.ncols, w, (uint32_t)rows_pad, (T *)xs_use);
                }
            } else if constexpr (WIDE8) {
                if (threads > 0)
                    hipLaunchKernelGGL(k_slice_pack_widen8, dim3((unsigned)((threads + 255) / 256)), dim3(256), 0, st, (const int8_t *)X, ldx,
                                       (uint32_t)p.ncols, w, nslices, (int16_t *)xs_use, (uint32_t)rows_pad, (const uint32_t *)p.lds_col_order);
            } else if constexpr (EL8) {
                const uint64_t th8 = (uint64_t)p.ncols * nslices * 32;
                if (th8 > 0)
                    hipLaunchKernelGGL((k_slice_pack<T, 2, 5>), dim3((unsigned)((th8 + 255) / 256)), dim3(256), 0, st, X, ldx,
                                       (uint32_t)p.ncols, w, nslices, (T *)xs_use, (uint32_t)rows_pad, (const uint32_t *)p.lds_col_order);
            } else if (threads > 0) {
                hipLaunchKernelGGL((k_slice_pack<T, PVEC, 4>), dim3((unsigned)((threads + 255) / 256)), dim3(256), 0, st, X, ldx,
                                   (uint32_t)p.ncols, w, nslices, (T *)xs_use, (uint32_t)rows_pad, (const uint32_t *)p.lds_col_order);
            }
        }
    }
    LdsArgs a{};
    a.tok = p.lds_tok;
    a.tiles = p.lds_tiles;
    a.rowmap = p.lds_rowmap;
    a.xs = (const char *)xs_use;
    a.c = (char *)C;
    a.slice_stride = rows_pad * ROWB;
    a.ldc_bytes = (uint32_t)((size_t)ldc * (((WIDE8 || sizeof(T) == 2) && deq_amax) ? 4 : sizeof(T)));
    a.w = w_lanes;
    a.nslices = nslices;
    a.ntiles = p.lds_ntiles;
    a.accumulate = accumulate ? 1 : 0;
    const uint32_t S = p.lds_col_splits;
    const uint64_t ldp = split16 ? (uint64_t)w_lanes * 2 : (uint64_t)w_lanes * 4 / sizeof(T);
    const size_t part_es = split16 ? 2 : sizeof(T);
    const uint64_t lds_rows = p.lds_rows ? p.lds_rows : (uint64_t)p.nrows;
    const bool deq_at_reduce = S > 1 && deq_amax != nullptr;
    if (S > 1) {
        const size_t need = (((size_t)S * (size_t)lds_rows * ldp * part_es + 255) & ~(size_t)255) + (size_t)p.lds_tail_nseg * nslices * 64 * 8;
        if (int rc = ensure(&g->scratch, &g->scratch_bytes, std::max<size_t>(need, 256))) return rc;
        a.c = (char *)g->scratch;
        a.ldc_bytes = (uint32_t)(ldp * part_es);
        a.accumulate = 0;
    }
    const uint32_t *kernel_amax = (deq_at_reduce || split16) ? nullptr : deq_amax;
    a.wdelta = p.lds_wdelta;
    a.deq_amax = kernel_amax;
    a.deq_log2 = deq_log2;
    a.post_mul = kernel_amax ? g->post_mul : nullptr;
    a.post_add = kernel_amax ? g->post_add : nullptr;
    a.post_relu = kernel_amax ? g->post_relu : 0;
    a.xcd_group = (nslices == 1 || nslices == 2 || nslices == 4 || nslices == 8) ? 8 / nslices : 0;
    a.xcd_sx = 1;
    if (a.xcd_group && p.lds_is_code && nslices > 1) {
        uint32_t sx = (uint32_t)std::max<int64_t>(0, g_tune.lds_xcd_slices);
        if (sx == 0) {
            const uint64_t nchunks = ((uint64_t)p.ncols + p.lds_kc - 1) / std::max(1u, p.lds_kc);
            const double fill = p.lds_ntiles && nchunks ? (double)p.lds_slots / ((double)p.lds_ntiles * (double)nchunks) : 1.0;
            sx = fill < 0.3 ? std::min(nslices, 4u) : (EL8 ? 1u : 2u);
        }
        if (sx > 1 && sx <= nslices && nslices % sx == 0) {
            a.xcd_sx = sx;
            a.xcd_group *= sx;
        }
    }
    a.half_split = HS ? 1u : 0u;
    a.xcd_contig = (a.xcd_group && p.lds_contig_tiles) ? (p.lds_ntiles + a.xcd_group - 1) / a.xcd_group : 0;
    const uint32_t grid = a.xcd_group ? 8 * ((p.lds_ntiles + a.xcd_group - 1) / a.xcd_group) * a.xcd_sx : p.lds_ntiles * nslices;
    using KernelFn = void (*)(LdsArgs);
    KernelFn fn = nullptr;
    const bool long16 = p.lds_nw == 16 && p.lds_batch == LDS_L16_BATCH;
    if (p.lds_is_code) {
        if (!g_tune.lds_code || g_tune.lds_ablate) return fail(PYGIM_ERR_INVALID, "this group's LDS plan is a code stream: lds_code was switched off (or lds_ablate on) after it was created");
        const bool w8 = p.lds_nw == 8;
        if constexpr (EL8) {
            if (!w8 || kernel_amax || S > 1 || p.lds_row_bytes != 512) return fail(PYGIM_ERR_INVALID, "internal: 8-byte LDS-staged product on an unsupported plan");
            if constexpr (std::is_same<T, double>::value) fn = k_lds_code8_f64;
            else fn = k_lds_code8_i64;
        } else if constexpr (sizeof(T) == 1) {
            if (!w8 || (accumulate && S <= 1)) return fail(PYGIM_ERR_INVALID, "internal: INT8 LDS-staged product on an unsupported plan");
            fn = split16 ? k_lds_code8_i16 : kernel_amax ? k_lds_code8_i8_deq : k_lds_code8_i8;
        } else if constexpr (sizeof(T) == 2) {
            if ((kernel_amax || split16) && !w8) return fail(PYGIM_ERR_INVALID, "internal: dequantising LDS-staged product on an unsupported plan");
            fn = kernel_amax ? k_lds_code8_i16_deq : (w8 ? k_lds_code8_i16 : k_lds_code_i16);
        } else if constexpr (std::is_same<T, float>::value) {
            fn = kernel_amax ? (w8 ? k_lds_code8_f32_deq : k_lds_code_f32_deq) : (w8 ? k_lds_code8_f32 : k_lds_code_f32);
        } else {
            fn = kernel_amax ? (w8 ? k_lds_code8_i32_deq : k_lds_code_i32_deq) : (w8 ? k_lds_code8_i32 : k_lds_code_i32);
        }
        if (g_tune.lds_stamp && fn == k_lds_code8_f32) {
            fn = k_lds_code8_f32_ts;
            a.stamps = (uint64_t *)(uintptr_t)g_tune.lds_stamp;
        }
        a.code = p.lds_code;
        a.code_start = p.lds_code_start;
        a.piece_bytes = p.lds_code_piece;
    } else if constexpr (sizeof(T) == 1 || sizeof(T) == 8) {
        return fail(PYGIM_ERR_INVALID, "internal: the INT8 / INT64 / DBL64 LDS-staged product exists in the code-stream form only");
    } else if (kernel_amax) {
        if (p.lds_nw != 16 || p.lds_wdelta || sizeof(T) != 4) return fail(PYGIM_ERR_INVALID, "internal: dequantising LDS-staged product on an unsupported plan");
        if constexpr (std::is_same<T, float>::value) fn = long16 ? k_lds_spmm_f32_w16b_deq : k_lds_spmm_f32_w16_deq;
        else if constexpr (std::is_same<T, int32_t>::value) fn = long16 ? k_lds_spmm_i32_w16b_deq : k_lds_spmm_i32_w16_deq;
    } else if constexpr (sizeof(T) == 2) {
        if (p.lds_nw != 16) return fail(PYGIM_ERR_INVALID, "internal: INT16 LDS-staged product needs the 16-wave plan");
        fn = long16 ? k_lds_spmm_i16_w16b : (p.lds_wdelta ? k_lds_spmm_i16_w16_val : k_lds_spmm_i16_w16);
    } else if (long16) {
        if constexpr (std::is_same<T, float>::value) fn = k_lds_spmm_f32_w16b;
        else fn = k_lds_spmm_i32_w16b;
    } else if constexpr (std::is_same<T, float>::value) {
        fn = p.lds_nw == 16 ? (p.lds_wdelta ? k_lds_spmm_f32_w16_val : k_lds_spmm_f32_w16) : k_lds_spmm_f32_w8;
#ifdef PYGIM_LDS_ABLATE
        if (p.lds_nw == 16 && !p.lds_wdelta && !long16) {
            switch (g_tune.lds_ablate) {
                case 6: fn = k_lds_spmm_f32_w16_ab6; break;
                case 7: fn = k_lds_spmm_f32_w16_ab7; break;
                case 10: fn = k_lds_spmm_f32_w16_ab10; break;
                case 11: fn = k_lds_spmm_f32_w16_ab11; break;
                case 12: fn = k_lds_spmm_f32_w16_ab12; break;
                case 15: fn = k_lds_spmm_f32_w16_ab15; break;
                case 16: fn = k_lds_spmm_f32_w16_ab16; break;
                case 17: fn = k_lds_spmm_f32_w16_ab17; break;
                case 18: fn = k_lds_spmm_f32_w16_ab18; break;
                case 19: fn = k_lds_spmm_f32_w16_ab19; break;
                default: break;
            }
        }
#else
        if (g_tune.lds_ablate) return fail(PYGIM_ERR_INVALID, "lds_ablate needs the ablation build (make -C pygim_amd/csrc ablate)");
#endif
    } else {
        fn = p.lds_nw == 16 ? (p.lds_wdelta ? k_lds_spmm_i32_w16_val : k_lds_spmm_i32_w16) : k_lds_spmm_i32_w8;
    }
    if (kernel_amax && g_tune.lds_ablate) return fail(PYGIM_ERR_INVALID, "lds_ablate is a timing experiment of the plain kernel");
    if (!fn) return fail(PYGIM_ERR_INVALID, "internal: no LDS-staged kernel for this plan");
    {
        static std::set<std::pair<int, KernelFn>> attr_done;
        int dev = 0;
        HIP_TRY(hipGetDevice(&dev));
        std::lock_guard<std::mutex> lk(g_ctx.mu);
        if (!attr_done.count({dev, fn})) {
            HIP_TRY(hipFuncSetAttribute((const void *)fn, hipFuncAttributeMaxDynamicSharedMemorySize, (int)LDS_BYTES));
            attr_done.insert({dev, fn});
        }
    }
    hipLaunchKernelGGL(fn, dim3(grid), dim3(p.lds_nw * 64), LDS_BYTES, st, a);
    g->lds_runs++;
    if (split16 && lds_rows > 0 && w > 0) {
        const uint64_t total = lds_rows * w;
        const dim3 rg((unsigned)((total + 255) / 256));
        if (!deq_amax)
            hipLaunchKernelGGL((k_lds_reduce16<0>), rg, dim3(256), 0, st, (const int16_t *)g->scratch, S, lds_rows, w, ldp, (void *)C, ldc, accumulate ? 1 : 0, nullptr, 0, nullptr, nullptr, 0);
        else if (WIDE8)
            hipLaunchKernelGGL((k_lds_reduce16<1>), rg, dim3(256), 0, st, (const int16_t *)g->scratch, S, lds_rows, w, ldp, (void *)C, ldc, 0, deq_amax, deq_log2, g->post_mul, g->post_add, g->post_relu);
        else
            hipLaunchKernelGGL((k_lds_reduce16<2>), rg, dim3(256), 0, st, (const int16_t *)g->scratch, S, lds_rows, w, ldp, (void *)C, ldc, 0, deq_amax, deq_log2, g->post_mul, g->post_add, g->post_relu);
    } else if (S > 1 && lds_rows > 0 && w > 0 && sizeof(T) == 4 && (w & 3) == 0 && (ldp & 3) == 0 && (ldc & 3) == 0 && ((uintptr_t)C & 15) == 0) {
        if constexpr (sizeof(T) == 4) {
            const uint64_t total4 = lds_rows * (w >> 2);
            const dim3 rg((unsigned)((total4 + 255) / 256));
            if (deq_at_reduce)
                hipLaunchKernelGGL((k_lds_reduce_v4<T, true>), rg, dim3(256), 0, st, (const T *)g->scratch, S, lds_rows, w, ldp, (void *)C, ldc, 0, deq_amax, deq_log2, g->post_mul,
                                   g->post_add, g->post_relu);
            else
                hipLaunchKernelGGL((k_lds_reduce_v4<T, false>), rg, dim3(256), 0, st, (const T *)g->scratch, S, lds_rows, w, ldp, (void *)C, ldc, accumulate ? 1 : 0, nullptr, 0, nullptr,
                                   nullptr, 0);
        }
    } else if (S > 1 && lds_rows > 0 && w > 0) {
        const uint64_t total = lds_rows * w;
        if constexpr (sizeof(T) == 4) {
            if (deq_at_reduce)
                hipLaunchKernelGGL((k_lds_reduce_deq<T>), dim3((unsigned)((total + 255) / 256)), dim3(256), 0, st, (const T *)g->scratch, S, lds_rows, w, ldp, (float *)C, ldc,
                                   deq_amax, deq_log2, g->post_mul, g->post_add, g->post_relu);
        }
        if (!deq_at_reduce)
            hipLaunchKernelGGL((k_lds_reduce<T>), dim3((unsigned)((total + 255) / 256)), dim3(256), 0, st, (const T *)g->scratch, S, lds_rows, w, ldp, C,
                               ldc, accumulate ? 1 : 0);
    }
    if (lds_rows < (uint64_t)p.nrows && w > 0) {
        if constexpr (sizeof(T) == 4) {
            using A = typename AccOf<T>::type;
            if (!p.lds_tail_segs || !p.lds_tail_rowseg) return fail(PYGIM_ERR_INVALID, "internal: an LDS plan that leaves rows out has no segment table for them");
            const uint32_t ntail = (uint32_t)((uint64_t)p.nrows - lds_rows);
            const size_t split_bytes = S > 1 ? (((size_t)S * (size_t)lds_rows * ldp * sizeof(T) + 255) & ~(size_t)255) : 0;
            const size_t park_bytes = (size_t)p.lds_tail_nseg * nslices * 64 * sizeof(A);
            if (int rc = ensure(&g->scratch, &g->scratch_bytes, std::max<size_t>(split_bytes + park_bytes, 256))) return rc;
            A *parked = (A *)((char *)g->scratch + split_bytes);
            if (p.lds_tail_nseg > 0)
                hipLaunchKernelGGL((k_lds_tail_seg<T>), dim3(p.lds_tail_nseg, nslices), dim3(512), 0, st, p.lds_tail_segs, p.lds_tail_nseg, p.colind, (const char *)xs_use,
                                   (uint64_t)(rows_pad * ROWB), parked);
            const int64_t ldc_b = (int64_t)ldc * 4;
            if (deq_amax)
                hipLaunchKernelGGL((k_lds_tail_fin<T, true>), dim3(ntail, nslices), dim3(64), 0, st, p.lds_tail_rowseg, (uint32_t)lds_rows, parked, w, (void *)C, ldc_b, 0, deq_amax,
                                   deq_log2, g->post_mul, g->post_add, g->post_relu);
            else
                hipLaunchKernelGGL((k_lds_tail_fin<T, false>), dim3(ntail, nslices), dim3(64), 0, st, p.lds_tail_rowseg, (uint32_t)lds_rows, parked, w, (void *)C, ldc_b,
                                   accumulate ? 1 : 0, nullptr, 0, nullptr, nullptr, 0);
        } else {
            return fail(PYGIM_ERR_INVALID, "internal: an LDS plan that leaves rows to the tail kernels exists for 4-byte element types only");
        }
    }
    kt.stop();
    HIP_TRY(hipGetLastError());
    return 0;
}

template <typename T> bool want_lds(const Group *g, const Part &p, uint32_t w, int64_t ldc, const void *C, bool accumulate = false) {
    if constexpr (sizeof(T) == 8) {
        if (!p.lds_is_code || p.lds_nw != 8 || p.lds_row_bytes != 512 || p.lds_col_splits > 1 || false) return false;
    } else if (p.lds_row_bytes == 512) return false;
    if constexpr (sizeof(T) == 1) {
        if (!p.lds_is_code || p.lds_nw != 8 || (accumulate && p.lds_col_splits <= 1)) return false;
        if ((int64_t)(w / 2) < g_tune.lds_min_width) return false;
    }
    if constexpr (sizeof(T) == 2) {
        if ((w & 1) || (ldc & 1) || ((uintptr_t)C & 3) || (p.lds_nw != 16 && !p.lds_is_code)) return false;
    }
    if (!p.lds_tiles || g_tune.lds_mode == 2 || (!p.lds_is_code && (p.vals != nullptr) != (p.lds_wdelta != 0)) || g->deq_out || g->pre_xs) return false;
    if (p.lds_half && (sizeof(T) != 4 || w > 32)) return false;
    if (p.lds_is_code && (!g_tune.lds_code || g_tune.lds_ablate)) return false;
    if (g_tune.lds_mode == 0 && (g_tune.panel_mode == 1 || g_tune.csr_kernel != 0 || g_tune.force_vec_bytes != 0)) return false;
    if (sizeof(T) > 1 && (int64_t)(sizeof(T) == 8 ? (size_t)w : (size_t)w * sizeof(T) / 4) < (sizeof(T) == 8 ? g_tune.lds_min_width8 : g_tune.lds_min_width)) return false;
    if ((uint64_t)ldc * sizeof(T) >= (1ull << 32)) return false;
    return true;
}

template <typename T>
int launch_block(Group *g, Part &p, const void *X, int64_t ldx, void *C, int64_t ldc, int64_t w, bool accumulate,
                 hipStream_t st) {
    const T *x = (const T *)X;
    T *c = (T *)C;
    const uint32_t ww = (uint32_t)w;
    if (want_lds<T>(g, p, ww, ldc, C, accumulate)) return launch_lds<T>(g, p, x, ldx, c, ldc, ww, accumulate, st);
    if (ww <= 4 && g_tune.vec_kernel && g_tune.force_vec_bytes == 0 && g_tune.csr_kernel == 0 && p.rowptr && p.nrows > 0) {
        using A = typename AccOf<T>::type;
        constexpr size_t LDS_TOTAL = 160 * 1024 - 64;
        const size_t panel_lds = (((((size_t)p.panel_cols + 1) * ww * sizeof(T)) + 15) & ~(size_t)15) + 16;
        const size_t per_entry = 4 + (size_t)ww * sizeof(A);
        const bool lds_rule = g_tune.vec_lds && g_tune.panel_mode != 2 && p.d_items && p.col16 && p.lp_panel.n_tasks == 0 && !p.panel_locality_used &&
                              p.npanels >= 1 && p.panel_long128.size() == 4 * (size_t)p.npanels && (uint64_t)p.nnz < (1ull << 31) &&
                              (double)p.nnz >= (double)g_tune.vec_lds_min_seg * (double)p.nrows * (double)p.npanels;
        if (lds_rule && panel_lds + 64 * 12 * per_entry <= LDS_TOTAL) {
            const size_t stage_budget = std::min<size_t>(32 * 1024, LDS_TOTAL - panel_lds);
            uint32_t F16 = (uint32_t)(stage_budget / (64 * per_entry)) / 24 * 24;
            const int merge4 = F16 == 0 ? 1 : 0;
            if (merge4) F16 = (uint32_t)(stage_budget / (64 * per_entry)) / 12 * 12;
            const size_t shmem = panel_lds + 64 * (size_t)F16 * per_entry;
            const uint32_t cu = (uint32_t)std::max(g_ctx.cu_count, 1);
            if (!p.d_spmv_units) {
                std::vector<uint32_t> act;
                double wsum = 0;
                for (uint32_t q = 0; q < p.npanels; q++)
                    if (p.panel_off[q + 1] > p.panel_off[q]) {
                        act.push_back(q);
                        wsum += (double)std::max<uint64_t>(p.panel_nnz[q], p.panel_off[q + 1] - p.panel_off[q]);
                    }
                if (!act.empty()) {
                    std::vector<uint32_t> nb(act.size(), 1);
                    if (act.size() < cu) {
                        uint32_t left = cu - (uint32_t)act.size();
                        std::vector<std::pair<double, size_t>> rem;
                        uint32_t given = 0;
                        for (size_t k = 0; k < act.size(); k++) {
                            const uint32_t q = act[k];
                            const double share = (double)left * (double)std::max<uint64_t>(p.panel_nnz[q], p.panel_off[q + 1] - p.panel_off[q]) / wsum;
                            const uint32_t fl = (uint32_t)share;
                            nb[k] += fl;
                            given += fl;
                            rem.emplace_back(share - fl, k);
                        }
                        std::sort(rem.begin(), rem.end(), [](const std::pair<double, size_t> &x, const std::pair<double, size_t> &y) { return x.first > y.first; });
                        for (size_t k = 0; given < left && k < rem.size(); k++, given++) nb[rem[k].second]++;
                    }
// ... 154 lines not shown
```

### pygim_amd/csrc/rt_plans.inc

```
template <typename T> void launch_check_ones(const void *v, uint32_t n, int *flag, hipStream_t st) {
    hipLaunchKernelGGL((k_check_ones<T>), dim3((n + 255) / 256), dim3(256), 0, st, (const T *)v, n, flag);
}

void plan_long_rows(const uint32_t *rowptr, int64_t nrows, uint32_t thresh, uint32_t seg, const std::vector<char> *flags,
                    std::vector<uint32_t> &tasks, std::vector<uint32_t> &desc) {
    for (int64_t r = 0; r < nrows; r++) {
        const uint32_t s = rowptr[r], e = rowptr[r + 1];
        const bool is_long = flags ? (*flags)[(size_t)r] != 0 : (e - s > thresh);
        if (!is_long || e == s) continue;
        const uint32_t first = (uint32_t)(tasks.size() / 3);
        uint32_t n = 0;
        for (uint32_t a = s; a < e; a += seg, n++) {
            tasks.push_back((uint32_t)r);
            tasks.push_back(a);
            tasks.push_back(std::min(e, a + seg));
        }
        desc.push_back((uint32_t)r);
        desc.push_back(first);
        desc.push_back(n);
    }
}

int build_lds_plan(Part &p, size_t es, int *d_flag_sorted, hipStream_t st, const std::vector<uint32_t> &h_rowptr, int64_t h_hint);
double now_ms();
// ... 426 lines not shown
    };
    const size_t val_es = es;
    const bool int8_code = es == 1 && t_plan_dtype == PYGIM_INT8 && allow_code && g_tune.lds_code && g_tune.lds_waves == 16 && g_tune.lds_code_waves != 16;
    if (es == 1) {
        if (!int8_code) return 0;
        es = 2;
    }
    const bool el8_code = es == 8 && (t_plan_dtype == PYGIM_INT64 || t_plan_dtype == PYGIM_DBL64) && allow_code && g_tune.lds_code &&
                          g_tune.lds_waves == 16 && g_tune.lds_code_waves != 16;
    if (es == 8 && !el8_code) return 0;
    if (g_tune.lds_mode == 2 || (es != 4 && es != 2 && es != 8) || p.is_extra || p.nnz == 0 || p.nrows == 0 || p.ncols == 0) return 0;
    if ((p.vals || es == 2) && g_tune.lds_waves != 16) return 0;
    if (h_hint > 0 && (es == 8 ? h_hint : (h_hint * (int64_t)std::max<size_t>(es, 2)) / 4) < (es == 8 ? g_tune.lds_min_width8 : g_tune.lds_min_width)) return 0;
    if ((uint64_t)p.ncols * (es == 8 ? 512ull : 256ull) >= (1ull << 32) - (1ull << 20) || (uint64_t)p.nnz >= (1ull << 31)) return 0;
    LdsGeometry geo;
    geo.NW = g_tune.lds_waves == 16 ? 16 : 8;
    geo.KA = lds_ka(geo.NW);
    geo.KC = LDS_KC;
    geo.BATCH = lds_batch(geo.NW);
    geo.keep_tile_order = p.lds_contig_tiles ? 1u : 0u;
    const bool want_code = allow_code && g_tune.lds_code && geo.NW == 16 &&
                           ((es == 4 && t_plan_dtype == PYGIM_FLT32) || (es == 4 && t_plan_dtype == PYGIM_INT32) ||
                            (es == 2 && t_plan_dtype == PYGIM_INT16) || int8_code || el8_code);
    const int64_t slice_b = es == 8 ? 512 : 256;
    const int64_t nsl_hint = h_hint > 0 ? (h_hint * (int64_t)es + slice_b - 1) / slice_b : 4;
    if (want_code) {
        const int64_t cw = g_tune.lds_code_waves;
        const bool eight = cw == 8 || (cw != 16 && LDS_CODE_AUTO_WAVES == 8) || int8_code || el8_code;
        if (eight) {
            geo.NW = 8;
            geo.KA = el8_code ? LDS_CODE8_KA64 : LDS_CODE8_KA;
            geo.BATCH = 8;
        }
        if (el8_code) geo.row_bytes = 512;
    }
    if (g_tune.lds_round_tiles && h_hint > 0)
        geo.rows_per_tile = lds_rows_per_tile((uint32_t)p.nrows, geo.NW * geo.KA, (uint32_t)nsl_hint, (uint32_t)std::max(g_ctx.cu_count, 1));
    const bool f32_split_ok = g_tune.lds_col_split_f32 == 1 ? p.nnz >= (1 << 20) : g_tune.lds_col_split_f32 != 0;
    uint32_t rows_lds = (uint32_t)p.nrows;
    if (g_tune.lds_col_split != 1 && (geo.NW == 16 || want_code) && !el8_code && (t_plan_dtype != PYGIM_FLT32 || f32_split_ok) && !p.vals) {
        const uint32_t cus = (uint32_t)std::max(g_ctx.cu_count, 1);
        const uint64_t nsl = h_hint > 0 ? (uint64_t)nsl_hint : 1;
        const uint64_t tall = ((uint64_t)p.nrows + geo.NW * geo.KA - 1) / (geo.NW * geo.KA), wgs = tall * nsl;
        uint32_t S = 1;
        if (g_tune.lds_col_split > 1) S = (uint32_t)std::min<int64_t>(g_tune.lds_col_split, 16);
        else if (wgs * 2 <= cus) S = (uint32_t)std::min<uint64_t>(8, cus / wgs);
        if (g_tune.lds_col_split == 0 && g_tune.lds_row_tail > 0 && want_code && es == 4 && !p.lds_forced && (uint64_t)p.nrows * 8 < (1ull << 31)) {
            const uint64_t full = (uint64_t)geo.NW * geo.KA;
            for (uint32_t S2 = 8; S2 > S; S2--) {
                const uint64_t tall2 = cus / (nsl * S2);
                if (!tall2) continue;
                const uint64_t covered = tall2 * full;
                if (covered >= (uint64_t)p.nrows) break;
                if (((uint64_t)p.nrows - covered) * 100 <= (uint64_t)p.nrows * (uint64_t)g_tune.lds_row_tail && tall2 * nsl * S2 * 10 >= (uint64_t)cus * 9) {
                    S = S2;
                    rows_lds = (uint32_t)covered;
                    break;
                }
            }
        }
        if (S > 1 && (uint64_t)p.nrows * S < (1ull << 31)) {
            geo.col_splits = S;
            geo.rows_per_tile = 0;
            if (g_tune.lds_split_order && (((uint64_t)rows_lds + geo.NW * geo.KA - 1) / (geo.NW * geo.KA)) * nsl * S <= cus) geo.keep_tile_order = 1;
            if (g_tune.lds_col_split == 0 && g_tune.lds_fill_tiles && rows_lds == (uint32_t)p.nrows) {
                const uint64_t tall2 = cus / (nsl * S);
                if (tall2 > tall && tall2 <= 2 * tall) geo.rows_per_tile = (uint32_t)std::max<uint64_t>(16, ((uint64_t)p.nrows + tall2 - 1) / tall2);
            }
        }
    }
    if (want_code) {
        code_ring(geo.NW, geo.row_bytes, geo.NBUF, geo.KC);
        geo.boundary = g_tune.lds_code_boundary == 2 ? 0u : 1u;
    }
    const int64_t lanes_hint = h_hint > 0 ? (h_hint * (int64_t)es + 3) / 4 : 0;
    const bool half = want_code && g_tune.lds_half_split && es == 4 && geo.NW == 8 && !p.vals && !p.lds_forced && lanes_hint > 0 && lanes_hint <= 32 &&
                      (t_plan_dtype == PYGIM_INT32 || (t_plan_dtype == PYGIM_FLT32 && f32_split_ok)) && rows_lds == (uint32_t)p.nrows && (uint64_t)p.ncols >= 4ull * geo.KC &&
                      !g_tune.lds_code_exp && !(g_tune.lds_fail & 7);
    uint32_t half_H = 0;
    if (half) {
        half_H = (uint32_t)(((((uint64_t)p.ncols + 1) / 2 + geo.KC - 1) / geo.KC) * geo.KC);
        geo.half_split = 1;
    }
    const bool narrow_hint = es != 8 && lanes_hint > 0 && lanes_hint <= 32;
    const double min_reuse_x100 = !narrow_hint ? (double)g_tune.lds_min_reuse_x100
                                               : std::max((double)g_tune.lds_min_reuse_x100, (double)g_tune.lds_min_reuse_narrow_x100 * (half ? 1.6 : 1.0));
    if (g_tune.lds_mode == 0 && !p.lds_forced &&
        lds_plan_uniform_reuse((uint64_t)p.nnz, (uint32_t)p.nrows, half ? half_H : (uint32_t)p.ncols, geo) * 100.0 < min_reuse_x100)
        return 0;
    if (p.cols_sorted < 0) {
        int unsorted = 0;
        if (hipMemsetAsync(d_flag_sorted, 0, sizeof(int), st) != hipSuccess) return fail(PYGIM_ERR_HIP, "flag reset");
        hipLaunchKernelGGL(k_check_sorted_cols, dim3((unsigned)((p.nrows + 255) / 256)), dim3(256), 0, st, p.rowptr, p.colind,
                           (uint32_t)p.nrows, d_flag_sorted);
        if (hipMemcpy(&unsorted, d_flag_sorted, sizeof(int), hipMemcpyDeviceToHost) != hipSuccess) return fail(PYGIM_ERR_HIP, "sortedness check");
        p.cols_sorted = unsorted ? 0 : 1;
    }
    if (!p.cols_sorted) return 0;
    const uint32_t code_op = t_plan_dtype == PYGIM_FLT32 ? 0x02000000u : t_plan_dtype == PYGIM_INT32 ? 0x68000000u : t_plan_dtype == PYGIM_DBL64 ? LDS_CODE_ADD_F64 :
                             t_plan_dtype == PYGIM_INT64 ? LDS_CODE_ADD_U64 : LDS_CODE_PK_ADD_U16;
    std::vector<uint32_t> rorder;
    if (want_code && p.nrows == p.ncols && rows_lds == (uint32_t)p.nrows && !half &&
        (g_tune.lds_tile_order == 1 || p.lds_forced || (g_tune.lds_tile_order == 2 && p.nnz >= (1 << 20)))) {
        find_similarity(p, st, g_tune.lds_tile_order == 1 || p.lds_forced);
        if (p.sim_kind == 2) {
            rorder = p.sim_order;
            p.lds_tile_labels = p.sim_labels;
            p.lds_tile_largest = p.sim_largest;
        }
        lap("similarity order (label propagation)");
    }
    const uint32_t *ro = rorder.empty() ? nullptr : rorder.data();
    std::string dev_why;
    if (want_code && g_tune.lds_codegen && !(g_tune.lds_fail & 7) && !g_tune.lds_code_exp) {
        CgDeviceResult dr;
        std::string exec_why;
        auto alloc_exec = [&](size_t bytes) -> void * { return exec_alloc(bytes, &exec_why); };
        auto free_exec = [&](void *q) { (void)hsa_amd_memory_pool_free(q); };
        uint32_t *d_vals32 = nullptr;
        if (p.vals && val_es < 4) {
            if (hipMalloc((void **)&d_vals32, std::max<size_t>((size_t)p.nnz * 4, 256)) != hipSuccess) {
                (void)hipGetLastError();
                d_vals32 = nullptr;
            } else if (val_es == 1) hipLaunchKernelGGL((k_widen_vals<int8_t>), dim3((unsigned)(((uint64_t)p.nnz + 255) / 256)), dim3(256), 0, st, (const int8_t *)p.vals, (uint64_t)p.nnz, d_vals32);
            else hipLaunchKernelGGL((k_widen_vals<int16_t>), dim3((unsigned)(((uint64_t)p.nnz + 255) / 256)), dim3(256), 0, st, (const int16_t *)p.vals, (uint64_t)p.nnz, d_vals32);
        }
        struct FreeVals { uint32_t *q; ~FreeVals() { if (q) (void)hipFree(q); } } free_vals{d_vals32};
        g_cg_fail_big_alloc = (g_tune.lds_fail & 8) != 0;
        dev_why = (p.vals && val_es < 4 && !d_vals32) ? std::string("out of device memory for the widened values") :
                  cg_run_on_device(p.rowptr, p.colind, es == 8 ? nullptr : (p.vals && val_es < 4) ? d_vals32 : (const uint32_t *)p.vals, es == 8 ? (const uint64_t *)p.vals : nullptr, h_rowptr.data(), ro, rows_lds,
                                   half ? half_H : (uint32_t)p.ncols, geo, code_op,
                                   (uint32_t)std::max<int64_t>(0, g_tune.lds_code_gsize), (uint32_t)std::max<int64_t>(0, g_tune.lds_code_nsets), st, alloc_exec,
                                   free_exec, dr, [] { return now_ms(); }, half ? half_H : 0u);
        if (dev_why.empty()) {
            if (plan_timing)
                fprintf(stderr, "[pygim plan] device code generation: rows %.1f, chunk lists %.1f, keys + sort %.1f, columns %.1f, slots + groups %.1f, sizes %.1f, emission %.1f, "
                                "whole %.1f ms (%.1f MB of code)\n", dr.ms[0], dr.ms[1], dr.ms[2], dr.ms[3], dr.ms[4], dr.ms[5], dr.ms[6], dr.ms[7], dr.code_bytes / 1e6);
            if (g_tune.lds_codegen == 2) {
                std::string diff = codegen_verify(p, geo, code_op, h_rowptr, ro, dr, d_vals32, rows_lds, half ? half_H : 0u);
                if (!diff.empty()) {
                    (void)hsa_amd_memory_pool_free(dr.code);
                    (void)hipFree(dr.d_start);
                    (void)hipFree(dr.d_rowmap);
                    (void)hipFree(dr.d_tiles);
                    return fail(PYGIM_ERR_INVALID, ("lds_codegen = 2: the device-generated code stream differs from the host encoder's: " + diff).c_str());
                }
            }
            p.lds_code = (char *)dr.code;
            p.lds_code_bytes = dr.code_bytes;
            p.lds_code_start = dr.d_start;
            p.lds_rowmap = dr.d_rowmap;
            p.lds_tiles = dr.d_tiles;
            p.lds_code_pairs = dr.pairs;
            p.lds_code_shared = dr.shared;
            p.lds_is_code = true;
            p.lds_code_piece = geo.KC * geo.row_bytes / geo.NW;
            p.lds_code_gsize = dr.regs.gsize;
            p.lds_code_nsets = dr.regs.nsets;
            p.lds_col_splits = geo.col_splits;
            p.lds_kc = geo.KC;
            p.lds_nbuf = geo.NBUF;
            p.lds_row_bytes = geo.row_bytes;
            p.lds_ka = geo.KA;
            p.lds_ntiles = dr.ntiles;
            p.lds_nw = geo.NW;
            p.lds_batch = geo.BATCH;
            p.lds_slots = dr.slots;
            p.lds_tokens = dr.entries;
            p.lds_codegen_device = true;
            p.lds_rows = rows_lds < (uint32_t)p.nrows ? rows_lds : 0;
            p.lds_half = half ? half_H : 0;
            lap("code stream generated on the device");
            return build_tail_segments(p, h_rowptr);
        }
        (void)hipGetLastError();
        if (plan_timing) fprintf(stderr, "[pygim plan] device code generation not used: %s\n", dev_why.c_str());
        p.lds_codegen_why = dev_why;
    } else if (want_code) {
        p.lds_codegen_why = !g_tune.lds_codegen ? "lds_codegen = 0" : (g_tune.lds_fail & 7) ? "lds_fail set" : "timing experiment";
    }
    std::vector<uint32_t> h_col((size_t)p.nnz);
    if (hipMemcpy(h_col.data(), p.colind, h_col.size() * 4, hipMemcpyDeviceToHost) != hipSuccess) return fail(PYGIM_ERR_HIP, "colind D2H");
    lap("sortedness check + column ids D2H");
    std::vector<uint32_t> h_val;
    std::vector<uint64_t> h_val64;
    if (p.vals) {
        h_val.resize((size_t)p.nnz);
        if (es == 4) {
            if (hipMemcpy(h_val.data(), p.vals, h_val.size() * 4, hipMemcpyDeviceToHost) != hipSuccess) return fail(PYGIM_ERR_HIP, "values D2H");
        } else if (es == 8) {
            h_val64.resize((size_t)p.nnz);
            if (hipMemcpy(h_val64.data(), p.vals, h_val64.size() * 8, hipMemcpyDeviceToHost) != hipSuccess) return fail(PYGIM_ERR_HIP, "values D2H");
            for (size_t i = 0; i < h_val.size(); i++) h_val[i] = (uint32_t)i;
        } else if (val_es == 1) {
            std::vector<int8_t> v8((size_t)p.nnz);
            if (hipMemcpy(v8.data(), p.vals, v8.size(), hipMemcpyDeviceToHost) != hipSuccess) return fail(PYGIM_ERR_HIP, "values D2H");
            for (size_t i = 0; i < v8.size(); i++) h_val[i] = (uint32_t)(int32_t)v8[i];
        } else {
            std::vector<uint16_t> v16((size_t)p.nnz);
            if (hipMemcpy(v16.data(), p.vals, v16.size() * 2, hipMemcpyDeviceToHost) != hipSuccess) return fail(PYGIM_ERR_HIP, "values D2H");
            for (size_t i = 0; i < v16.size(); i++) h_val[i] = want_code ? (uint32_t)(int32_t)(int16_t)v16[i] : (uint32_t)v16[i] * 0x10001u;
        }
    }
    LdsPlanHost plan;
    try {
        if (g_tune.lds_fail & 4) throw std::runtime_error("lds_fail: forced failure of the schedule build");
        if (half) half_split_virtual_matrix(h_rowptr, (uint32_t)p.nrows, half_H, h_col, h_val);
        lds_plan_build(h_rowptr.data(), h_col.data(), rows_lds, half ? half_H : (uint32_t)p.ncols, geo, plan, (unsigned)std::max<int64_t>(0, g_tune.lds_threads),
                       (p.vals || half) ? h_val.data() : nullptr, ro);
    } catch (const std::exception &e) {
        p.lds_note = std::string("the schedule of the LDS-staged product could not be built (") + e.what() + "): the L2 sweep serves this group";
        return 0;
    }
    lap("schedule (tiles, tokens)");
    if (geo.NW == 16 && !p.vals && !want_code && g_tune.lds_long_slots && plan.slots > 0 &&
        (double)plan.ntokens / ((double)plan.slots * geo.NW) >= (double)g_tune.lds_long_slots) {
        LdsGeometry gl = geo;
        gl.KA = LDS_L16_KA;
        gl.BATCH = LDS_L16_BATCH;
        gl.rows_per_tile = geo.col_splits > 1 ? 0 : g_tune.lds_round_tiles && h_hint > 0
                               ? lds_rows_per_tile((uint32_t)p.nrows, gl.NW * gl.KA, (uint32_t)nsl_hint, (uint32_t)std::max(g_ctx.cu_count, 1))
                               : 0;
        const uint32_t r_now = geo.rows_per_tile ? geo.rows_per_tile : geo.NW * geo.KA, r_new = gl.rows_per_tile ? gl.rows_per_tile : gl.NW * gl.KA;
        if (r_new >= r_now) {
            try {
                lds_plan_build(h_rowptr.data(), h_col.data(), (uint32_t)p.nrows, (uint32_t)p.ncols, gl, plan,
                               (unsigned)std::max<int64_t>(0, g_tune.lds_threads), nullptr);
            } catch (const std::exception &e) {
                p.lds_note = std::string("the schedule of the LDS-staged product could not be built (") + e.what() + "): the L2 sweep serves this group";
                return 0;
            }
            geo = gl;
        }
    }
    std::vector<uint32_t>().swap(h_col);
    std::vector<uint32_t>().swap(h_val);
    if (p.vals && !want_code) {
        if ((uint64_t)plan.tok.size() * 8 >= (1ull << 32)) return 0;
        p.lds_wdelta = (uint32_t)(plan.tok.size() * 4);
        plan.tok.insert(plan.tok.end(), plan.wts.begin(), plan.wts.end());
        std::vector<uint32_t>().swap(plan.wts);
    }
    auto up = [&](auto **dst, const auto &v) {
        using E = typename std::remove_reference<decltype(v[0])>::type;
        const size_t bytes = std::max<size_t>(v.size() * sizeof(E), 64);
        if (hipMalloc((void **)dst, bytes) != hipSuccess) return false;
        return v.empty() || hipMemcpy(*dst, v.data(), v.size() * sizeof(E), hipMemcpyHostToDevice) == hipSuccess;
    };
    if (plan.header_overflow) {
        p.lds_note = "the LDS-staged schedule does not fit its slot headers (more than 16 383 batches of one wave in one chunk, or more than 5 M columns): the L2 sweep serves this group";
        return 0;
    }
    if (want_code) {
        LdsCodeHost ch;
        try {
            if (g_tune.lds_fail & 1) throw std::runtime_error("lds_fail: forced failure of the code generation");
            lds_code_from_plan(plan, t_plan_dtype == PYGIM_FLT32 ? 0x02000000u : t_plan_dtype == PYGIM_INT32 ? 0x68000000u : t_plan_dtype == PYGIM_DBL64 ? LDS_CODE_ADD_F64 :
                                     t_plan_dtype == PYGIM_INT64 ? LDS_CODE_ADD_U64 : LDS_CODE_PK_ADD_U16, ch,
                               (unsigned)std::max<int64_t>(0, g_tune.lds_threads), (uint32_t)std::max<int64_t>(0, g_tune.lds_code_gsize),
                               (uint32_t)std::max<int64_t>(0, g_tune.lds_code_nsets), (uint32_t)std::max<int64_t>(0, g_tune.lds_code_exp),
                               h_val64.empty() ? nullptr : h_val64.data());
        } catch (const std::exception &e) {
            p.lds_note = std::string("code-stream form not available: generating the instruction streams failed (") + e.what() + ")";
            return -1;
        }
        lap("code generation");
        std::vector<uint32_t>().swap(plan.tok);
        std::string why_exec;
        void *code = (g_tune.lds_fail & 2) ? nullptr : exec_alloc_upload(ch.code.data(), ch.code.size() * 4, &why_exec);
        if (!code) {
            p.lds_note = "code-stream form not available: " + (why_exec.empty() ? std::string("lds_fail: forced failure of the executable allocation") : why_exec) +
                         " (" + std::to_string(ch.code.size() * 4) + " bytes of code)";
            return -1;
        }
        if (!up(&p.lds_code_start, ch.start) || !up(&p.lds_rowmap, plan.rowmap) || !up(&p.lds_tiles, plan.tiles)) {
            (void)hsa_amd_memory_pool_free(code);
            return fail(PYGIM_ERR_HIP, "code-stream plan upload");
        }
        lap("code + tables upload");
        p.lds_code = (char *)code;
        p.lds_code_bytes = ch.code.size() * 4;
        p.lds_code_pairs = ch.pairs;
        p.lds_is_code = true;
        p.lds_code_piece = geo.KC * geo.row_bytes / geo.NW;
        p.lds_code_gsize = ch.regs.gsize;
        p.lds_code_nsets = ch.regs.nsets;
        p.lds_code_shared = ch.shared;
    } else if (!up(&p.lds_tok, plan.tok) || !up(&p.lds_rowmap, plan.rowmap) || !up(&p.lds_tiles, plan.tiles)) {
        return fail(PYGIM_ERR_HIP, "LDS plan upload");
    }
    p.lds_col_splits = geo.col_splits;
    p.lds_rows = rows_lds < (uint32_t)p.nrows ? rows_lds : 0;
    p.lds_half = half ? half_H : 0;
    p.lds_kc = geo.KC;
    p.lds_nbuf = geo.NBUF;
    p.lds_row_bytes = geo.row_bytes;
    p.lds_ka = geo.KA;
    p.lds_ntiles = plan.ntiles;
    p.lds_nw = geo.NW;
    p.lds_batch = geo.BATCH;
    p.lds_slots = plan.slots;
    p.lds_tokens = plan.ntokens;
    return build_tail_segments(p, h_rowptr);
}

double now_ms() {
    using namespace std::chrono;
    return duration<double, std::milli>(steady_clock::now().time_since_epoch()).count();
}

int need_init() {
    if (!g_ctx.inited) return fail(PYGIM_ERR_NO_DEVICE, "backend not initialised: call dpu_init_ranks / pygim_init_ranks first");
    return 0;
}
```

### pygim_amd/csrc/rt_state.inc

```
thread_local std::string g_err;
int fail(int code, const std::string &msg) {
    g_err = msg;
    return code;
}
#define HIP_TRY(expr)                                                                          \
    do {                                                                                       \
        hipError_t _e = (expr);                                                                \
        if (_e != hipSuccess) {                                                                \
            (void)hipGetLastError();                                                           \
            return fail(PYGIM_ERR_HIP, std::string(#expr) + ": " + hipGetErrorString(_e));     \
        }                                                                                      \
    } while (0)

size_t dtype_size(int dt) {
    switch (dt) {
        case PYGIM_INT8: return 1;
        case PYGIM_INT16: return 2;
        case PYGIM_INT32: return 4;
        case PYGIM_INT64: return 8;
        case PYGIM_FLT32: return 4;
        case PYGIM_DBL64: return 8;
    }
    return 0;
}

struct Tunables {
    int64_t long_row_threshold = 4096;
    int64_t long_segment = 512;
    int64_t force_vec_bytes = 0;
    int64_t csr_kernel = 0;
    int64_t coo_chunk = 512;
    int64_t coo_via_rowptr = 0;
    int64_t panel_mode = 0;
    int64_t panel_bytes = 4 << 20;
    int64_t panel_min_seg = 8;
    int64_t panel_block = 256;
    int64_t panel_lds_pad = 0;
    int64_t panel_coop = 512;
    int64_t panel_pack = 1;
    int64_t slice_group_bytes = 640ll << 20;
    int64_t vec_kernel = 1;
    int64_t vec_lds = 1;
    int64_t vec_lds_min_seg = 14;
    int64_t merge_parts = 1;
    int64_t narrow_vals = 1;
    int64_t split_unit_pattern = 1;
    int64_t panel_locality = 1;
    int64_t panel_col16 = 1;
    int64_t fuse_windows = 1;
    int64_t host_windows = 0;
    int64_t host_direct = 1;
    int64_t kernel_events = 0;
    int64_t lds_mode = 0;
    int64_t lds_min_reuse_x100 = 75;
    int64_t lds_min_width = 5;
    int64_t lds_min_width8 = 33;
    int64_t lds_min_reuse_narrow_x100 = 75;
    int64_t lds_threads = 0;
    int64_t lds_waves = 16;
    int64_t lds_long_slots = 128;
    int64_t lds_code = 1;
    int64_t lds_col_split = 0;
    int64_t lds_col_split_f32 = 1;
    int64_t lds_row_tail = 3;
    int64_t lds_half_split = 1;
    int64_t lds_direct_x = 1;
    int64_t lds_split_order = 1;
    int64_t lds_fill_tiles = 1;
    int64_t lds_code_nbuf = 0;
    int64_t lds_code_waves = 0;
    int64_t lds_code_kc = 0;
    int64_t lds_code_gsize = 0;
    int64_t lds_code_nsets = 0;
    int64_t lds_round_tiles = 1;
    int64_t lds_tile_order = 2;
    int64_t lds_lp_rounds = 12;
    int64_t lds_codegen = 1;
    int64_t lds_xcd_slices = 0;
    int64_t lds_code_boundary = 0;
    int64_t lds_code_exp = 0;
    int64_t lds_hybrid = 1;
    int64_t lds_hybrid_contig = 1;
    int64_t lds_hybrid_min = 128;
    int64_t lds_stamp = 0;
    int64_t lds_fail = 0;
    int64_t lds_ablate = 0;
} g_tune;

struct LongPlan {
    uint32_t n_long = 0, n_tasks = 0, thresh = 0;
    uint32_t *d_tasks = nullptr;
    uint32_t *d_desc = nullptr;
};

struct Part {
    int64_t nrows = 0, ncols = 0, nnz = 0;
    uint32_t *rowptr = nullptr;
    uint32_t *rowind = nullptr;
    uint32_t *colind = nullptr;
    void *vals = nullptr;
    void *vals_narrow = nullptr;
    bool own_rowptr = false, own_rowind = false, own_colind = false, own_vals = false;
    LongPlan lp_base, lp_panel;
    uint32_t *d_items = nullptr;
    size_t n_items = 0;
    std::vector<size_t> panel_off;
    std::vector<uint32_t> panel_coop;
    uint32_t npanels = 0, panel_cols = 0;
    unsigned short *col16 = nullptr;
    std::vector<uint32_t> panel_long128;
    std::vector<uint64_t> panel_nnz;
    SpmvUnit *d_spmv_units = nullptr;
    uint32_t n_spmv_units = 0;
    std::vector<int64_t> dense_cols;
    std::unique_ptr<Part> extra;
    std::unique_ptr<Part> hy_dense, hy_sparse;
    bool lds_forced = false;
    bool lds_contig_tiles = false;
    uint32_t *lds_col_order = nullptr;
    std::string hy_note;
    uint32_t *lds_tok = nullptr, *lds_nb = nullptr, *lds_chunks = nullptr, *lds_rowmap = nullptr;
    LdsTile *lds_tiles = nullptr;
    int cols_sorted = -1;
    uint32_t lds_ntiles = 0, lds_nw = 8, lds_batch = 8, lds_wdelta = 0;
    char *lds_code = nullptr;
    uint64_t *lds_code_start = nullptr;
    uint64_t lds_code_bytes = 0, lds_code_pairs = 0;
    uint32_t lds_rows = 0;
    uint32_t lds_half = 0;
    uint32_t *lds_tail_segs = nullptr;
    uint32_t *lds_tail_rowseg = nullptr;
    uint32_t lds_tail_nseg = 0;
    uint32_t lds_col_splits = 1;
    uint32_t lds_code_piece = 0;
    uint32_t lds_kc = 0, lds_nbuf = 0;
    uint32_t lds_row_bytes = 256, lds_ka = 0;
    uint32_t lds_code_gsize = 0, lds_code_nsets = 0;
    uint64_t lds_code_shared = 0;
    std::string lds_note;
    bool lds_codegen_device = false;
    bool panel_locality_used = false;
    int sim_kind = -1;
    std::vector<uint32_t> sim_order;
    uint32_t sim_labels = 0, sim_largest = 0;
    double sim_agree = 0.0;
    std::string sim_why;
    uint32_t lds_tile_labels = 0, lds_tile_largest = 0;
    std::string lds_codegen_why;
    bool lds_is_code = false;
    uint64_t lds_slots = 0, lds_tokens = 0;
    bool is_extra = false;
    bool no_pack = false;
    bool timed = false;
};

struct Group {
    int format = 0, dtype = 0;
    int64_t h = 0, total_rows = 0, total_cols = 0;
    std::vector<Part> parts;
    std::unique_ptr<Part> merged;
    bool all_ones = true;
    void *scratch = nullptr;
    size_t scratch_bytes = 0;
    void *stage_in = nullptr;
    size_t stage_in_bytes = 0;
    void *stage_out = nullptr;
    size_t stage_out_bytes = 0;
    void *xq = nullptr;
    size_t xq_bytes = 0;
    void *oq = nullptr;
    size_t oq_bytes = 0;
    const void *packed_src = nullptr;
    void *packed_buf = nullptr;
    int64_t packed_ld = 0, packed_w = 0;
    bool x_unchanged = false;
    int64_t serial = 0;
    int64_t lds_runs = 0;
    const void *pre_xs = nullptr;
    float *deq_out = nullptr;
    int64_t deq_ld = 0;
    const uint32_t *deq_amax = nullptr;
    int deq_log2 = 0;
    const float *post_mul = nullptr, *post_add = nullptr;
    int post_relu = 0;
    void **h_ptrs = nullptr;
    size_t h_ptrs_n = 0;
    hipEvent_t ev_ptrs[2] = {nullptr, nullptr};
    int ptr_slot = 0;
    void *xcat = nullptr;
    size_t xcat_bytes = 0;
    void **d_ptrs = nullptr;
    size_t d_ptrs_n = 0;
    int *d_flags = nullptr;
    hipStream_t side = nullptr;
    hipEvent_t ev_fork = nullptr, ev_join = nullptr;
    hipStream_t pipe_up = nullptr, pipe_down = nullptr;
    std::vector<hipEvent_t> pipe_ev;
    int64_t host_windows_used = 0;
    int64_t host_direct_used = 0;
    bool host_copies_slow = false;
    double timers[5] = {0, 0, 0, 0, 0};
    std::vector<std::pair<hipEvent_t, hipEvent_t>> ev_pending;
    bool kernel_events = false;
    double ev_ms = 0;
    int64_t ev_count = 0;
};

struct Context {
    bool inited = false;
    int device = 0;
    int cu_count = 0;
    int64_t nr_ranks = 0;
    std::set<Group *> groups;
    std::mutex mu;
    struct XsBuf {
        void *ptr = nullptr;
// ... 150 lines not shown
            fp->found = true;
            return HSA_STATUS_INFO_BREAK;
        }
        return HSA_STATUS_SUCCESS;
    }, &fp);
    if (!fp.found) return nullptr;
    ep.agent = f.agent;
    ep.pool = fp.pool;
    ep.ok = true;
    return &ep;
}
static void *exec_alloc(size_t bytes, std::string *why = nullptr) {
    auto say = [&](const char *m) { if (why) *why = m; };
    int dev = 0;
    if (hipGetDevice(&dev) != hipSuccess) { say("no current HIP device"); return nullptr; }
    ExecPool *ep;
    {
        std::lock_guard<std::mutex> lk(g_ctx.mu);
        ep = exec_pool_locked(dev);
    }
    if (!ep) { say("the HSA runtime offers no executable device memory pool"); return nullptr; }
    void *ptr = nullptr;
    if (hsa_amd_memory_pool_allocate(ep->pool, bytes, HSA_AMD_MEMORY_POOL_EXECUTABLE_FLAG, &ptr) != HSA_STATUS_SUCCESS) {
        say("the executable pool could not allocate the code");
        return nullptr;
    }
    return ptr;
}
static void *exec_alloc_upload(const void *host, size_t bytes, std::string *why = nullptr) {
    auto say = [&](const char *m) { if (why) *why = m; };
    const size_t piece = std::min<size_t>(bytes, (size_t)64 << 20);
    void *ptr = exec_alloc(bytes, why), *stage = nullptr;
    if (!ptr) return nullptr;
    if (hipMalloc(&stage, std::max<size_t>(piece, 256)) != hipSuccess) {
        (void)hipGetLastError();
        (void)hsa_amd_memory_pool_free(ptr);
        say("out of device memory for the staging buffer of the code upload");
        return nullptr;
    }
    bool ok = true;
    for (size_t off = 0; off < bytes && ok; off += piece) {
        const size_t nb = std::min(piece, bytes - off);
        ok = hipMemcpy(stage, (const char *)host + off, nb, hipMemcpyHostToDevice) == hipSuccess;
        const uint64_t n16 = nb / 16;
        if (ok && n16) {
            hipLaunchKernelGGL(k_copy16, dim3((unsigned)((n16 + 255) / 256)), dim3(256), 0, 0, (const u32x4_t *)stage, (u32x4_t *)((char *)ptr + off), n16);
            ok = hipGetLastError() == hipSuccess && hipDeviceSynchronize() == hipSuccess;
        }
    }
    (void)hipFree(stage);
    if (!ok) {
        (void)hsa_amd_memory_pool_free(ptr);
        say("copying the code to the device failed");
        return nullptr;
    }
    return ptr;
}

void free_part(Part &p) {
    if (p.own_rowptr && p.rowptr) (void)hipFree(p.rowptr);
    if (p.own_rowind && p.rowind) (void)hipFree(p.rowind);
    if (p.own_colind && p.colind) (void)hipFree(p.colind);
    if (p.own_vals && p.vals) (void)hipFree(p.vals);
    if (p.vals_narrow) (void)hipFree(p.vals_narrow);
    p.vals_narrow = nullptr;
    for (LongPlan *lp : {&p.lp_base, &p.lp_panel}) {
        if (lp->d_tasks) (void)hipFree(lp->d_tasks);
        if (lp->d_desc) (void)hipFree(lp->d_desc);
    }
    if (p.d_items) (void)hipFree(p.d_items);
    if (p.col16) (void)hipFree(p.col16);
    if (p.d_spmv_units) (void)hipFree(p.d_spmv_units);
    for (void *q : {(void *)p.lds_tok, (void *)p.lds_nb, (void *)p.lds_chunks, (void *)p.lds_rowmap, (void *)p.lds_tiles})
        if (q) (void)hipFree(q);
    p.lds_tok = p.lds_nb = p.lds_chunks = p.lds_rowmap = nullptr;
    p.lds_tiles = nullptr;
    if (p.lds_code) (void)hsa_amd_memory_pool_free(p.lds_code);
    if (p.lds_code_start) (void)hipFree(p.lds_code_start);
    p.lds_code = nullptr;
    p.lds_code_start = nullptr;
    p.lds_is_code = false;
    p.lds_row_bytes = 256;
    p.lds_col_splits = 1;
    p.lds_rows = 0;
    p.lds_half = 0;
    if (p.lds_tail_segs) (void)hipFree(p.lds_tail_segs);
    if (p.lds_tail_rowseg) (void)hipFree(p.lds_tail_rowseg);
    p.lds_tail_segs = p.lds_tail_rowseg = nullptr;
    p.lds_tail_nseg = 0;
    if (p.extra) free_part(*p.extra);
    if (p.hy_dense) free_part(*p.hy_dense);
    if (p.hy_sparse) free_part(*p.hy_sparse);
    if (p.lds_col_order) {
        std::lock_guard<std::mutex> lk(g_ctx.mu);
        for (auto &kv : g_ctx.xs_bufs)
            if (kv.second.order == (const void *)p.lds_col_order) { kv.second.src = nullptr; kv.second.order = nullptr; }
        (void)hipFree(p.lds_col_order);
    }
    p.lds_col_order = nullptr;
}

void free_group(Group *g) {
    for (auto &p : g->parts) free_part(p);
    if (g->merged) free_part(*g->merged);
    if (g->scratch) (void)hipFree(g->scratch);
    if (g->stage_in) (void)hipFree(g->stage_in);
    if (g->stage_out) (void)hipFree(g->stage_out);
    if (g->xcat) (void)hipFree(g->xcat);
    if (g->xq) (void)hipFree(g->xq);
    if (g->oq) (void)hipFree(g->oq);
    if (g->d_ptrs) (void)hipFree(g->d_ptrs);
    if (g->h_ptrs) (void)hipHostFree(g->h_ptrs);
    for (hipEvent_t e : g->ev_ptrs)
        if (e) (void)hipEventDestroy(e);
    if (g->d_flags) (void)hipFree(g->d_flags);
    if (g->side) (void)hipStreamDestroy(g->side);
    for (hipEvent_t e : g->pipe_ev)
        if (e) (void)hipEventDestroy(e);
    if (g->ev_fork) (void)hipEventDestroy(g->ev_fork);
    if (g->ev_join) (void)hipEventDestroy(g->ev_join);
    for (auto &e : g->ev_pending) {
        (void)hipEventDestroy(e.first);
        (void)hipEventDestroy(e.second);
    }
    delete g;
}

Group *lookup(int64_t handle) {
    Group *g = reinterpret_cast<Group *>(static_cast<uintptr_t>(handle));
    std::lock_guard<std::mutex> lk(g_ctx.mu);
    return g_ctx.groups.count(g) ? g : nullptr;
}
```

Measured before the change: 28760.

## Stream X row-major with run-time stride in LDS codegen, skipping slice-major pack

Adds a run-time-stride DMA path to the generated LDS code kernels. When the column-split plan qualifies, the kernels read X directly from the caller's row-major matrix instead of first running a slice-major pack copy. This removes the pack kernel and its extra pass over X. In exchange the DMA uses strided per-piece addressing with more scalar instructions per chunk, and a cost model decides when it pays off. New kernel variants (_rs) are referenced, and the tail kernel takes a stride parameter.

```diff
diff --git a/pygim_amd/autotune.py b/pygim_amd/autotune.py
--- a/pygim_amd/autotune.py
+++ b/pygim_amd/autotune.py
@@ -19,6 +19,10 @@
 LDS_COL_SPLIT = True
 LDS_ROW_TAIL = 3
 TAIL_S = 30e-6
+LDS_ROWMAJOR = True
+LDS_RM_PACK_S_PER_BYTE = 298e-15
+LDS_RM_FILL_S_PER_CHUNK = 22e-9
+LDS_CHUNK_COLS = 128
 LDS_MIN_LANES = 5
 LDS_MIN_REUSE_NARROW = 0.75
 LDS_HALF_SPLIT = True
@@ -82,6 +86,9 @@
             tall = tall2
         per_wg = max(cols_x / split * LDS_NS_PER_COLUMN + nnz / tall / split * ns_entry, cols_x / split * LDS_NS_PER_COLUMN_FLOOR) * 1e-9
         reduce_s = (split + 1) * nrows * h * es / RATE_STREAM
+        chunks_wg = -(-(-(-ncols // LDS_CHUNK_COLS)) // split)
+        if LDS_ROWMAJOR and cols_x == ncols and h % 64 == 0 and chunks_wg * LDS_RM_FILL_S_PER_CHUNK <= ncols * h * es * LDS_RM_PACK_S_PER_BYTE:
+            pack_s -= ncols * h * es * LDS_RM_PACK_S_PER_BYTE - chunks_wg * LDS_RM_FILL_S_PER_CHUNK
         return per_wg + reduce_s + pack_s + 2 * LAUNCH + (TAIL_S if tail_rows else 0.0)
     rpt = lds_rows_per_tile(int(nrows), nsl)
     tiles = -(-int(nrows) // rpt)
diff --git a/pygim_amd/csrc/kernels.hpp b/pygim_amd/csrc/kernels.hpp
--- a/pygim_amd/csrc/kernels.hpp
+++ b/pygim_amd/csrc/kernels.hpp
@@ -827,7 +827,7 @@
 constexpr uint32_t LDS_TAIL_SEG = 256;
 template <typename T>
 __global__ __launch_bounds__(512) void k_lds_tail_seg(const uint32_t *__restrict__ segs, uint32_t nseg, const uint32_t *__restrict__ colind, const char *__restrict__ xs,
-                                                      uint64_t slice_stride, typename AccOf<T>::type *__restrict__ parked) {
+                                                      uint64_t slice_stride, typename AccOf<T>::type *__restrict__ parked, uint64_t row_stride = 256) {
     static_assert(sizeof(T) == 4, "4-byte element types");
     using A = typename AccOf<T>::type;
     __shared__ A partial[8][64];
@@ -844,7 +844,7 @@
     }
     T x[32];
 #pragma unroll
-    for (int k = 0; k < 32; k++) x[k] = cols[k] != 0xFFFFFFFFu ? *(const T *)(xsl + (uint64_t)cols[k] * 256) : (T)0;
+    for (int k = 0; k < 32; k++) x[k] = cols[k] != 0xFFFFFFFFu ? *(const T *)(xsl + (uint64_t)cols[k] * row_stride) : (T)0;
     A acc = 0;
 #pragma unroll
     for (int k = 0; k < 32; k++) acc = (A)(acc + to_acc<T>(x[k]));
diff --git a/pygim_amd/csrc/lds_codegen.hpp b/pygim_amd/csrc/lds_codegen.hpp
--- a/pygim_amd/csrc/lds_codegen.hpp
+++ b/pygim_amd/csrc/lds_codegen.hpp
@@ -26,6 +26,7 @@
     uint32_t nrows = 0, ncols = 0, nchunks = 0, ntiles = 0, nstreams = 0;
     uint32_t S = 1, row_tiles = 0;
     uint32_t col_bits = 1;
+    uint32_t stride_rt = 0;
     uint32_t half_H = 0;
     uint32_t x0 = 6, acc0 = 28, vbase0 = 1, vbase1 = 2, vbase2 = 3, vl16 = 4, vtouch = 4, vjunk = 5;
     uint32_t s_xs = 80, s_ldsw = 82, s_cb = 84, s_ret = 86, s_pa = 92;
@@ -61,6 +62,9 @@
     if ((geo.half_split != 0) != (half_H != 0)) throw std::runtime_error("lds codegen: a half-split plan names its H (and only such a plan does)");
     if (half_H && (valued || wide || half_H % geo.KC || ncols != half_H)) throw std::runtime_error("lds codegen: half-split plans are unit-weight plans of 4-byte types over H = whole chunks of virtual columns");
     P.half_H = half_H;
+    P.stride_rt = geo.x_stride_rt ? 1 : 0;
+    if (P.stride_rt && (!lds_code_stride_ok(geo, R) || (geo.KC / geo.NW) * geo.NW != geo.KC || P.pieces * 4 != geo.KC / geo.NW))
+        throw std::runtime_error("lds codegen: the run-time-stride DMA needs the 8-wave 256-byte geometry with v26 / v27 free");
     P.nrows = nrows; P.ncols = ncols;
     P.nchunks = (ncols + geo.KC - 1) / geo.KC;
     const uint32_t R_rows = geo.rows_per_tile ? std::min(geo.rows_per_tile, geo.NW * geo.KA) : geo.NW * geo.KA;
@@ -351,7 +355,35 @@
         e.since_touch = 0;
         e.vm_touch++;
     };
-    auto dma = [&](uint32_t cid, uint32_t buf) {
+    auto dma = [&](uint32_t cid, uint32_t buf) -> uint32_t {
+        if (P.stride_rt) {
+            uint32_t issued = 0;
+            e.op(0x92000000u | (LDS_CODE_S_MUL << 16) | (0xFFu << 8) | LDS_CODE_S_STRIDE, cid * P.KC);
+            e.op(0x96000000u | ((LDS_CODE_S_MUL + 1) << 16) | (0xFFu << 8) | LDS_CODE_S_STRIDE, cid * P.KC);
+            e.op(0x80000000u | (P.s_pa << 16) | (LDS_CODE_S_MUL << 8) | P.s_xs);
+            e.op(0x82000000u | ((P.s_pa + 1) << 16) | ((LDS_CODE_S_MUL + 1) << 8) | (P.s_xs + 1));
+            for (uint32_t i = 0; i < P.pieces; i++) {
+                const uint32_t rows = lds_code_piece_rows(cid, P.KC, P.NW, s % P.NW, i, P.ncols);
+                if (!rows) break;
+                if (i) {
+                    e.op(0x80000000u | (P.s_pa << 16) | (LDS_CODE_S_STEP << 8) | P.s_pa);
+                    s_addc0(P.s_pa + 1, P.s_pa + 1);
+                }
+                if (i % 4 == 0) {
+                    if (i) {
+                        s_add_lit(P.s_pa, P.s_pa, 0x1000);
+                        s_addc0(P.s_pa + 1, P.s_pa + 1);
+                    }
+                    s_add_lit(124 , P.s_ldsw, buf * P.chunk_bytes + (i / 4) * 0x1000);
+                    e.op(0xBF800000u);
+                }
+                if (rows < 4) e.op(0x91FE8000u | (128u + 16u * rows));
+                e.op(0xDDF48000u | ((i % 4) * 1024), (P.s_pa << 16) | LDS_CODE_V_RM);
+                if (rows < 4) e.op(0xBEFE01C1u);
+                issued++;
+            }
+            return issued;
+        }
         s_add_lit(P.s_pa, P.s_xs, cid * P.chunk_bytes);
         s_addc0(P.s_pa + 1, P.s_xs + 1);
         for (uint32_t i = 0; i < P.pieces; i++) {
@@ -365,14 +397,14 @@
             }
             e.op(0xDDF48000u | ((i % 4) * 1024), (P.s_pa << 16) | P.vl16);
         }
+        return P.pieces;
     };
     uint64_t dma_issued = 0;
     uint64_t landed_mark[16];
     for (int q = 0; q < 16; q++) landed_mark[q] = 0;
     auto vm_now = [&]() { return dma_issued + e.vm_touch; };
     auto dma_chunk = [&](uint32_t j) {
-        dma(chunk_ids[j], j % P.NBUF);
-        dma_issued += P.pieces;
+        dma_issued += dma(chunk_ids[j], j % P.NBUF);
         landed_mark[j & 15] = vm_now();
     };
     auto wait_landed = [&](uint32_t j) {
diff --git a/pygim_amd/csrc/lds_plan.hpp b/pygim_amd/csrc/lds_plan.hpp
--- a/pygim_amd/csrc/lds_plan.hpp
+++ b/pygim_amd/csrc/lds_plan.hpp
@@ -44,12 +44,14 @@
     uint32_t row_bytes = 256;
     uint32_t boundary = 0;
     uint32_t half_split = 0;
+    uint32_t x_stride_rt = 0;
     uint32_t NBUF = 2;
 };
 
 struct LdsPlanHost {
     LdsGeometry geo;
     uint32_t ntiles = 0, nchunks = 0;
+    uint32_t ncols = 0;
     uint64_t ntokens = 0;
     uint64_t slots = 0;
     std::vector<uint32_t> tok;
@@ -121,6 +123,7 @@
     out.geo = geo;
     out.ntiles = ntiles;
     out.nchunks = nchunks;
+    out.ncols = ncols;
     out.tiles.assign(ntiles, LdsTile());
     out.rowmap.assign((size_t)ntiles * RS, 0xFFFFFFFFu);
 
@@ -312,6 +315,14 @@
     while (r.x0 + r.nx() > r.acc0 && r.gsize > 2) r.gsize -= wide ? 1 : 2;
     return r;
 }
+constexpr uint32_t LDS_CODE_S_STRIDE = 88, LDS_CODE_S_STEP = 89, LDS_CODE_S_MUL = 90, LDS_CODE_V_RM = 27;
+inline bool lds_code_stride_ok(const LdsGeometry &geo, const LdsCodeRegs &R) {
+    return geo.NW == 8 && geo.row_bytes == 256 && !geo.half_split && R.x0 + R.nx() <= LDS_CODE_V_RM && R.acc0 > LDS_CODE_V_RM;
+}
+PYGIM_LDS_HD_INLINE uint32_t lds_code_piece_rows(uint32_t cid, uint32_t KC, uint32_t NW, uint32_t wv, uint32_t i, uint32_t ncols) {
+    const uint64_t r = (uint64_t)cid * KC + (uint64_t)wv * (KC / NW) + 4ull * i;
+    return r >= ncols ? 0u : (uint32_t)(ncols - r < 4 ? ncols - r : 4);
+}
 constexpr uint32_t LDS_CODE_AUTO_WAVES = 8, LDS_CODE8_AUTO_NBUF = 5;
 constexpr uint32_t LDS_CODE8_KA64 = 114;
 constexpr uint32_t LDS_CODE8_KA = 228;
@@ -368,6 +379,9 @@
     const uint32_t RPB = 65536 / RB;
     if ((KC * geo.NBUF + RPB - 1) / RPB > 3) throw std::runtime_error("lds code: the ring is larger than three 64 KiB blocks");
     const uint32_t ntiles = plan.ntiles;
+    const bool stride_rt = geo.x_stride_rt != 0;
+    if (stride_rt && (!lds_code_stride_ok(geo, R) || experiment || (KC / NW) * NW != KC || pieces * 4 != KC / NW || (geo.NBUF >= 3 && !geo.boundary)))
+        throw std::runtime_error("lds code: the run-time-stride DMA needs the 8-wave 256-byte geometry with v26 / v27 free, the boundary hand-off and no timing experiment");
     constexpr uint32_t TOUCH_EVERY_DW = 256;
 
     struct Emit {
@@ -410,7 +424,35 @@
             e.since_touch = 0;
             e.vm_touch++;
         };
-        auto dma = [&](uint32_t cid, uint32_t buf) {
+        auto dma = [&](uint32_t cid, uint32_t buf) -> uint32_t {
+            if (stride_rt) {
+                uint32_t issued = 0;
+                e.op(0x92000000u | (LDS_CODE_S_MUL << 16) | (0xFFu << 8) | LDS_CODE_S_STRIDE, cid * KC);
+                e.op(0x96000000u | ((LDS_CODE_S_MUL + 1) << 16) | (0xFFu << 8) | LDS_CODE_S_STRIDE, cid * KC);
+                e.op(0x80000000u | (Rr.s_pa << 16) | (LDS_CODE_S_MUL << 8) | Rr.s_xs);
+                e.op(0x82000000u | ((Rr.s_pa + 1) << 16) | ((LDS_CODE_S_MUL + 1) << 8) | (Rr.s_xs + 1));
+                for (uint32_t i = 0; i < pieces; i++) {
+                    const uint32_t rows = lds_code_piece_rows(cid, KC, NW, wv, i, plan.ncols);
+                    if (!rows) break;
+                    if (i) {
+                        e.op(0x80000000u | (Rr.s_pa << 16) | (LDS_CODE_S_STEP << 8) | Rr.s_pa);
+                        s_addc0(Rr.s_pa + 1, Rr.s_pa + 1);
+                    }
+                    if (i % 4 == 0) {
+                        if (i) {
+                            s_add_lit(Rr.s_pa, Rr.s_pa, 0x1000);
+                            s_addc0(Rr.s_pa + 1, Rr.s_pa + 1);
+                        }
+                        s_add_lit(124 , Rr.s_ldsw, buf * chunk_bytes + (i / 4) * 0x1000);
+                        e.op(0xBF800000u);
+                    }
+                    if (rows < 4) e.op(0x91FE8000u | (128u + 16u * rows));
+                    e.op(0xDDF48000u | ((i % 4) * 1024), (Rr.s_pa << 16) | LDS_CODE_V_RM);
+                    if (rows < 4) e.op(0xBEFE01C1u);
+                    issued++;
+                }
+                return issued;
+            }
             s_add_lit(Rr.s_pa, Rr.s_xs, cid * chunk_bytes);
             s_addc0(Rr.s_pa + 1, Rr.s_xs + 1);
             for (uint32_t i = 0; i < pieces; i++) {
@@ -424,6 +466,7 @@
                 }
                 if (!(experiment & 2)) e.op(0xDDF48000u | ((i % 4) * 1024), (Rr.s_pa << 16) | Rr.vl16);
             }
+            return (experiment & 2) ? 0u : pieces;
         };
         uint64_t at = (uint64_t)t.tokstart[wv] * B;
         const uint32_t NBUF = geo.NBUF;
@@ -432,8 +475,7 @@
         auto vm_now = [&]() { return dma_issued + e.vm_touch; };
         std::vector<uint64_t> landed_mark(t.nch + NBUF + 1, 0);
         auto dma_chunk = [&](uint32_t j) {
-            dma(plan.chunks[t.chunk_off + j], j % NBUF);
-            dma_issued += (experiment & 2) ? 0 : pieces;
+            dma_issued += dma(plan.chunks[t.chunk_off + j], j % NBUF);
             landed_mark[j] = vm_now();
         };
         const bool spread = (experiment & 4) && pieces <= 4 && !mid;
diff --git a/pygim_amd/csrc/pygim_hip.hip b/pygim_amd/csrc/pygim_hip.hip
--- a/pygim_amd/csrc/pygim_hip.hip
+++ b/pygim_amd/csrc/pygim_hip.hip
@@ -173,6 +173,9 @@
     else if (n == "lds_col_split") slot = &g_tune.lds_col_split;
     else if (n == "lds_col_split_f32") slot = &g_tune.lds_col_split_f32;
     else if (n == "lds_fill_tiles") slot = &g_tune.lds_fill_tiles;
+    else if (n == "lds_rowmajor") slot = &g_tune.lds_rowmajor;
+    else if (n == "lds_rm_pack_fs_per_byte") slot = &g_tune.lds_rm_pack_fs_per_byte;
+    else if (n == "lds_rm_fill_ps_per_chunk") slot = &g_tune.lds_rm_fill_ps_per_chunk;
     else if (n == "lds_row_tail") slot = &g_tune.lds_row_tail;
     else if (n == "lds_split_order") slot = &g_tune.lds_split_order;
     else if (n == "lds_half_split") slot = &g_tune.lds_half_split;
@@ -799,6 +802,9 @@
             if (g->parts[i].lds_note != g->parts[0].lds_note) text += "; part " + std::to_string(i) + ": " + g->parts[i].lds_note;
     }
     for (size_t i = 0; i < g->parts.size(); i++)
+        if (!g->parts[i].lds_x_form.empty()) text += (g->parts.size() > 1 ? "; part " + std::to_string(i) + ": " : std::string("; ")) + g->parts[i].lds_x_form;
+    if (g->merged && !g->merged->lds_x_form.empty()) text += "; " + g->merged->lds_x_form;
+    for (size_t i = 0; i < g->parts.size(); i++)
         if (!g->parts[i].hy_note.empty()) text += "; part " + std::to_string(i) + ": " + g->parts[i].hy_note;
     const size_t n = std::min<size_t>(text.size(), (size_t)cap - 1);
     std::memcpy(out, text.data(), n);
diff --git a/pygim_amd/csrc/rt_launch.inc b/pygim_amd/csrc/rt_launch.inc
--- a/pygim_amd/csrc/rt_launch.inc
+++ b/pygim_amd/csrc/rt_launch.inc
@@ -271,6 +271,32 @@
     KernelTimer kt(g, st, !p.is_extra || p.timed);
     XsPin pin;
     void *xs_use = const_cast<void *>(lds_xs);
+    bool x_rowmajor = false;
+    if (p.lds_stride_rt) {
+        int why = 0;
+        const uint64_t kc = std::max(1u, p.lds_kc), per_wg = (((uint64_t)p.ncols + kc - 1) / kc + p.lds_col_splits - 1) / std::max(1u, p.lds_col_splits);
+        const uint64_t x_bytes = (uint64_t)p.ncols * w * sizeof(T);
+        const uint64_t max_chunks = (uint64_t)((double)x_bytes * (double)std::max<int64_t>(0, g_tune.lds_rm_pack_fs_per_byte) / (1000.0 * (double)std::max<int64_t>(1, g_tune.lds_rm_fill_ps_per_chunk)));
+        if (sizeof(T) != 4 || HS) why = 1;
+        else if (!g_tune.lds_rowmajor) why = 2;
+        else if (lds_xs || deq_amax) why = 3;
+        else if (p.lds_col_order) why = 4;
+        else if (w % 64) why = 5;
+        else if (((uintptr_t)X & 15) || ((uint64_t)ldx * sizeof(T)) % 16 || (uint64_t)ldx * sizeof(T) >= (1ull << 30) || (uint64_t)ldx < w) why = 6;
+        else if (g_tune.lds_rowmajor == 1 && per_wg > max_chunks) why = 7;
+        x_rowmajor = why == 0;
+        if (p.lds_x_form_code != why + 1) {
+            static const char *const reasons[] = {"", "not a plain 4-byte product", "lds_rowmajor = 0", "the copy quantises the features", "the copy gathers X in the plan's column order",
+                                                  "the width is not a whole number of 64-lane slices", "X is not 16-byte aligned with a row stride of a multiple of 16 bytes",
+                                                  "its workgroups land more chunks than the copy costs"};
+            p.lds_x_form_code = why + 1;
+            p.lds_x_form = x_rowmajor ? "X streamed row-major from the caller's matrix (no slice-major copy; " + std::to_string(per_wg) + " chunks per workgroup, at most " +
+                                            std::to_string(max_chunks) + ")"
+                                      : std::string("X packed slice-major (k_slice_pack): ") + reasons[why] +
+                                            (why == 7 ? " (" + std::to_string(per_wg) + " chunks per workgroup, at most " + std::to_string(max_chunks) + ")" : std::string());
+        }
+        if (x_rowmajor) xs_use = const_cast<void *>((const void *)X);
+    }
     if (!xs_use && g_tune.lds_direct_x && nslices == 1 && !HS && !WIDE8 && !p.lds_col_order && (size_t)ldx * sizeof(T) == ROWB && (size_t)w * sizeof(T) == ROWB &&
         ((uintptr_t)X & 255) == 0) {
         void *base = nullptr;
@@ -340,7 +366,8 @@
     a.rowmap = p.lds_rowmap;
     a.xs = (const char *)xs_use;
     a.c = (char *)C;
-    a.slice_stride = rows_pad * ROWB;
+    a.slice_stride = x_rowmajor ? (uint64_t)ROWB : rows_pad * ROWB;
+    a.x_stride = x_rowmajor ? (uint32_t)((uint64_t)ldx * sizeof(T)) : ROWB;
     a.ldc_bytes = (uint32_t)((size_t)ldc * (((WIDE8 || sizeof(T) == 2) && deq_amax) ? 4 : sizeof(T)));
     a.w = w_lanes;
     a.nslices = nslices;
@@ -402,6 +429,12 @@
             fn = kernel_amax ? (w8 ? k_lds_code8_f32_deq : k_lds_code_f32_deq) : (w8 ? k_lds_code8_f32 : k_lds_code_f32);
         } else {
             fn = kernel_amax ? (w8 ? k_lds_code8_i32_deq : k_lds_code_i32_deq) : (w8 ? k_lds_code8_i32 : k_lds_code_i32);
+        }
+        if (p.lds_stride_rt) {
+            if (g_tune.lds_stamp) return fail(PYGIM_ERR_INVALID, "lds_stamp: this group's plan takes X's row stride at run time; create it with lds_rowmajor = 0 for the stamped build");
+            if (fn == k_lds_code8_f32) fn = k_lds_code8_f32_rs;
+            else if (fn == k_lds_code8_i32) fn = k_lds_code8_i32_rs;
+            else return fail(PYGIM_ERR_INVALID, "internal: a run-time-stride code stream on an unsupported product");
         }
         if (g_tune.lds_stamp && fn == k_lds_code8_f32) {
             fn = k_lds_code8_f32_ts;
@@ -502,7 +535,7 @@
             A *parked = (A *)((char *)g->scratch + split_bytes);
             if (p.lds_tail_nseg > 0)
                 hipLaunchKernelGGL((k_lds_tail_seg<T>), dim3(p.lds_tail_nseg, nslices), dim3(512), 0, st, p.lds_tail_segs, p.lds_tail_nseg, p.colind, (const char *)xs_use,
-                                   (uint64_t)(rows_pad * ROWB), parked);
+                                   (uint64_t)a.slice_stride, parked, (uint64_t)(x_rowmajor ? a.x_stride : ROWB));
             const int64_t ldc_b = (int64_t)ldc * 4;
             if (deq_amax)
                 hipLaunchKernelGGL((k_lds_tail_fin<T, true>), dim3(ntail, nslices), dim3(64), 0, st, p.lds_tail_rowseg, (uint32_t)lds_rows, parked, w, (void *)C, ldc_b, 0, deq_amax,
diff --git a/pygim_amd/csrc/rt_plans.inc b/pygim_amd/csrc/rt_plans.inc
--- a/pygim_amd/csrc/rt_plans.inc
+++ b/pygim_amd/csrc/rt_plans.inc
@@ -532,6 +532,11 @@
         half_H = (uint32_t)(((((uint64_t)p.ncols + 1) / 2 + geo.KC - 1) / geo.KC) * geo.KC);
         geo.half_split = 1;
     }
+    if (want_code && g_tune.lds_rowmajor && geo.col_splits > 1 && es == 4 && val_es == 4 && !p.vals && !half && geo.boundary && !g_tune.lds_code_exp &&
+        (t_plan_dtype == PYGIM_FLT32 || t_plan_dtype == PYGIM_INT32) &&
+        lds_code_stride_ok(geo, lds_code_regs(geo.NW, (uint32_t)std::max<int64_t>(0, g_tune.lds_code_gsize), (uint32_t)std::max<int64_t>(0, g_tune.lds_code_nsets), false)) &&
+        geo.KC % (4 * geo.NW) == 0)
+        geo.x_stride_rt = 1;
     const bool narrow_hint = es != 8 && lanes_hint > 0 && lanes_hint <= 32;
     const double min_reuse_x100 = !narrow_hint ? (double)g_tune.lds_min_reuse_x100
                                                : std::max((double)g_tune.lds_min_reuse_x100, (double)g_tune.lds_min_reuse_narrow_x100 * (half ? 1.6 : 1.0));
@@ -608,6 +613,7 @@
             p.lds_code_gsize = dr.regs.gsize;
             p.lds_code_nsets = dr.regs.nsets;
             p.lds_col_splits = geo.col_splits;
+            p.lds_stride_rt = geo.x_stride_rt != 0;
             p.lds_kc = geo.KC;
             p.lds_nbuf = geo.NBUF;
             p.lds_row_bytes = geo.row_bytes;
@@ -740,6 +746,7 @@
         return fail(PYGIM_ERR_HIP, "LDS plan upload");
     }
     p.lds_col_splits = geo.col_splits;
+    p.lds_stride_rt = want_code && geo.x_stride_rt != 0;
     p.lds_rows = rows_lds < (uint32_t)p.nrows ? rows_lds : 0;
     p.lds_half = half ? half_H : 0;
     p.lds_kc = geo.KC;
diff --git a/pygim_amd/csrc/rt_state.inc b/pygim_amd/csrc/rt_state.inc
--- a/pygim_amd/csrc/rt_state.inc
+++ b/pygim_amd/csrc/rt_state.inc
@@ -65,6 +65,9 @@
     int64_t lds_row_tail = 3;
     int64_t lds_half_split = 1;
     int64_t lds_direct_x = 1;
+    int64_t lds_rowmajor = 1;
+    int64_t lds_rm_pack_fs_per_byte = 298;
+    int64_t lds_rm_fill_ps_per_chunk = 22000;
     int64_t lds_split_order = 1;
     int64_t lds_fill_tiles = 1;
     int64_t lds_code_nbuf = 0;
@@ -132,6 +135,9 @@
     uint32_t *lds_tail_rowseg = nullptr;
     uint32_t lds_tail_nseg = 0;
     uint32_t lds_col_splits = 1;
+    bool lds_stride_rt = false;
+    int lds_x_form_code = 0;
+    std::string lds_x_form;
     uint32_t lds_code_piece = 0;
     uint32_t lds_kc = 0, lds_nbuf = 0;
     uint32_t lds_row_bytes = 256, lds_ka = 0;
@@ -448,6 +454,9 @@
     p.lds_is_code = false;
     p.lds_row_bytes = 256;
     p.lds_col_splits = 1;
+    p.lds_stride_rt = false;
+    p.lds_x_form.clear();
+    p.lds_x_form_code = 0;
     p.lds_rows = 0;
     p.lds_half = 0;
     if (p.lds_tail_segs) (void)hipFree(p.lds_tail_segs);
```

After: 28660. Within noise of the previous version (-0.3%).
